# lis-epfl/apg_trajectory_tracking

Measured on AMD Instinct MI355X. Metric: env-steps/sec (fwd+bwd through dynamics), quad horizon=10 batch=65536, higher is better.
Workload: dtype f32; 1 GPU; quadrotor concurrent rollout fwd+bwd (dynamics + quad_mpc_loss + adjoint), BASELINE configs[1]; batch_per_gpu=65536, global_batch=65536, horizon=10, layout=packed, buffer_sets=20, input_bytes_all_sets=587202560, grad_state0=False, loss_mode=deferred, launch=hip-graph replays of the K steps, <= 1000 steps per graph, replays=3, parallelism=batch-sharded x1, no data-path collective

## Files before the change

### apg_trajectory_tracking_amd/_capi.py

```python
import ctypes
import os

import torch

_HERE = os.path.dirname(os.path.abspath(__file__))
LIB_PATH = os.environ.get("APG_LIB") or os.path.join(_HERE, "csrc", "libapg_hip.so")

LAYOUT_SOA = 0
LAYOUT_AOS = 1
LAYOUT_PACKED = 2
MAX_HORIZON = 48
ROLLOUT_BLOCK = 64

_c_float_p = ctypes.c_void_p


class ApgQuadParams(ctypes.Structure):
    _fields_ = [
        ("mass", ctypes.c_float),
        ("kinv", ctypes.c_float * 3),
        ("inertia", ctypes.c_float * 3),
        ("gravity", ctypes.c_float * 3),
        ("trans_drag", ctypes.c_float * 3),
        ("rot_drag", ctypes.c_float * 3),
# ... 257 lines not shown
        _I, _P, _P],
    "apg_wing_learnt_step_bwd": [
        _P, _P, _F, ctypes.POINTER(ApgWingParams), ctypes.POINTER(ctypes.c_float),
        _I, _P, _P, _P, _P, _P, _P],
    "apg_wing_learnt_rollout_workspace_floats": [_I],
    "apg_wing_learnt_rollout_fwd_bwd": [
        _P, _P, _P, _F, ctypes.POINTER(ApgWingLearnt),
        ctypes.POINTER(ApgWingLossWeights), _I, _I, _I, _P, _P, _P, _P, _P, _P, _P],
    "apg_wing_learnt_fit_grad_count": [],
    "apg_wing_learnt_fit_workspace_floats": [_I],
    "apg_wing_learnt_fit_fwd_bwd": [
        _P, _P, _F, ctypes.POINTER(ApgWingLearnt), _P, ctypes.POINTER(ApgWingParams),
        _F, _I, _P, _P, _P, _P, _P],
    "apg_wing_mlp_closed_loop": [
        _P, _I, _P, _F, ctypes.POINTER(ApgWingParams), ctypes.POINTER(ctypes.c_float),
        ctypes.POINTER(ApgLearntResidual),
        ctypes.POINTER(ApgWingPolicy), ctypes.POINTER(ctypes.c_float),
        ctypes.POINTER(ctypes.c_float), _F, _I, _I, _I, _F, _F, _I, _P, _P, _P,
        _P, _P, _P, _P, _P],
    "apg_planes_gemm_workspace_floats": [_I, _I, _I, _I],
    "apg_planes_gemm_default_wgs": [_I, _I, _I, _I],
    "apg_planes_gemm_multi_workspace_floats": [ctypes.POINTER(ApgGemmProblem), _I],
    "apg_planes_gemm_multi": [ctypes.POINTER(ApgGemmProblem), _I, _P, _P],
    "apg_planes_gemm": [_P, _I, _I, _P, _P, _I, _I, _I, _I,
                        ctypes.c_longlong, _P, _I, _P, _I, _P, _P],
    "apg_wing_step_fwd": [_P, _P, _F, ctypes.POINTER(ApgWingParams), _I, _I,
                          _P, _P],
    "apg_wing_step_bwd": [_P, _P, _F, ctypes.POINTER(ApgWingParams), _I, _I,
                          _P, _P, _P, _P],
    "apg_wing_rollout_fwd_bwd": [
        _P, _P, _P, _F, ctypes.POINTER(ApgWingParams),
        ctypes.POINTER(ApgWingLossWeights), _I, _I, _I, _P, _P, _P, _P, _P,
        ctypes.POINTER(ApgDeferredLoss), _P],
    "apg_wing_rollout_fwd": [_P, _P, _F, ctypes.POINTER(ApgWingParams), _I,
                             _I, _I, _P, _P],
    "apg_wing_set_two_per_lane": [_I],
    "apg_cartpole_step_fwd": [_P, _P, _F, ctypes.POINTER(ApgCartpoleParams),
                              _I, _I, _P, _P],
    "apg_cartpole_step_bwd": [_P, _P, _F, ctypes.POINTER(ApgCartpoleParams),
                              _I, _I, _P, _P, _P, _P],
    "apg_cartpole_rollout_fwd_bwd": [
        _P, _P, _F, ctypes.POINTER(ApgCartpoleParams), _I, _I, _I, _P, _P,
        _P, _P, _P, _P],
    "apg_cartpole_rollout_fwd": [_P, _P, _F, ctypes.POINTER(ApgCartpoleParams),
                                 _I, _I, _I, _P, _P],
    "apg_cartpole_policy_workspace_floats": [],
    "apg_cartpole_mlp_closed_loop": [
        _P, _F, ctypes.POINTER(ApgCartpoleParams), ctypes.POINTER(ApgCartpolePolicy),
        _I, _I, _I, _F, _I, _P, _P, _P, _P, _P, _P, _P, _P],
    "apg_cartpole_learnt_param_count": [],
    "apg_cartpole_learnt_workspace_floats": [_I],
    "apg_cartpole_learnt_step_fwd": [_P, _P, _F, ctypes.POINTER(ApgCartpoleLearnt), _I,
                                     _P, _P],
    "apg_cartpole_learnt_step_bwd": [_P, _P, _F, ctypes.POINTER(ApgCartpoleLearnt), _I,
                                     _P, _P, _P, _P, _P, _P],
    "apg_cartpole_learnt_rollout_fwd_bwd": [
        _P, _P, _F, ctypes.POINTER(ApgCartpoleLearnt), _I, _I, _I, _P, _P, _P, _P, _P,
        _P],
    "apg_cartpole_learnt_mlp_closed_loop": [
        _P, _F, ctypes.POINTER(ApgCartpoleLearnt), ctypes.POINTER(ApgCartpolePolicy),
        _I, _I, _I, _F, _I, _P, _P, _P, _P, _P, _P, _P, _P],
    "apg_quad_mpc_solve": [
        _P, _P, _I, _F, ctypes.POINTER(ApgQuadParams),
        ctypes.POINTER(ApgQuadLossWeights), ctypes.POINTER(ApgQuadMpcOptions), _I, _I,
        _P, _P, _P, _P],
    "apg_quad_mpc_closed_loop": [
        ctypes.POINTER(ApgQuadFlight), _F, ctypes.POINTER(ApgQuadParams),
        ctypes.POINTER(ApgLearntResidual), ctypes.POINTER(ApgQuadParams),
        ctypes.POINTER(ApgQuadLossWeights), ctypes.POINTER(ApgQuadMpcOptions), _I, _I,
        _P, _P, _P],
    "apg_quad_mpc_workspace_floats": [],
    "apg_cartpole_mpc_solve": [
        _P, _P, _F, ctypes.POINTER(ApgCartpoleParams),
        ctypes.POINTER(ApgCartpoleMpcOptions), _I, _I, _P, _P, _P, _P],
    "apg_cartpole_mpc_closed_loop": [
        _P, _F, ctypes.POINTER(ApgCartpoleParams), ctypes.POINTER(ApgCartpoleLearnt),
        ctypes.POINTER(ApgCartpoleParams), ctypes.POINTER(ApgCartpoleMpcOptions),
        _I, _I, _I, _I, _F, _I, _P, _P, _P, _P, _P, _P, _P, _P],
    "apg_reduce_loss_partials": [_P, _I, _P, _P],
    "apg_loss_partials_count": [_I],
    "apg_stream_copy": [_P, _P, ctypes.c_longlong, _P],
    "apg_stream_copy_shape": [_P, _P, ctypes.c_longlong, _I, _P],
    "apg_stream_rows_probe": [_P, ctypes.c_longlong, _P, ctypes.c_longlong, _I, _P],
    "apg_version": [],
    "apg_last_error_string": [],
}
_RESTYPES = {"apg_last_error_string": ctypes.c_char_p,
             "apg_planes_gemm_multi_workspace_floats": ctypes.c_longlong,
             "apg_quad_mlp_step_partials_floats": ctypes.c_longlong,
             "apg_quad_mlp_rollout_step_partials_floats": ctypes.c_longlong,
             "apg_linear_wgrad_workspace_floats": ctypes.c_longlong}

_lib = None


def lib():
    global _lib
    if _lib is None:
        if not os.path.exists(LIB_PATH):
            raise RuntimeError(
                f"{LIB_PATH} not found: build it with "
                "`python -m apg_trajectory_tracking_amd.build` "
                "(there is no CPU / PyTorch fallback for the APG kernels)")
        handle = ctypes.CDLL(LIB_PATH)
        for name, argtypes in SIGNATURES.items():
            fn = getattr(handle, name)
            fn.argtypes = argtypes
            fn.restype = _RESTYPES.get(name, ctypes.c_int)
        _lib = handle
    return _lib


def check(code, what):
    if code != 0:
        msg = lib().apg_last_error_string().decode()
        exc = ValueError if code == -1 else RuntimeError
        raise exc(f"{what} failed ({code}): {msg}")


def ptr(t):
    return None if t is None else t.data_ptr()


def stream_of(t):
    return torch.cuda.current_stream(t.device).cuda_stream


def require_device(*tensors):
    dev = None
    for t in tensors:
        if t is None:
            continue
        if not t.is_cuda:
            raise RuntimeError(
                "apg_trajectory_tracking_amd kernels run on an MI355X only: "
                f"got a tensor on {t.device} (no CPU fallback exists)")
        if t.dtype != torch.float32:
            raise TypeError(f"fp32 tensors required, got {t.dtype}")
        if not t.is_contiguous():
            raise ValueError("contiguous tensors required")
        if dev is None:
            dev = t.device
        elif t.device != dev:
            raise RuntimeError("all tensors must live on the same device")
    return dev


def loss_partials_count(B):
    return 1 if B <= 0 else (B + ROLLOUT_BLOCK - 1) // ROLLOUT_BLOCK
```

### apg_trajectory_tracking_amd/csrc/apg_device.h

```cpp
#pragma once
#include <hip/hip_runtime.h>
#include <stdint.h>

#include "apg.h"

#if !defined(APG_EXPERIMENT_BUILD) &&                                          \
    (defined(APG_STAMP) || defined(APG_QX) || defined(APG_EXP_NO_STORES) ||    \
     defined(APG_TRIG_1WORD) || defined(APG_SW_TRIG) || defined(APG_MLP_EXP) || \
     defined(APG_ROWS_BLOCK) || defined(APG_ROWS_ACT_PRE) ||                   \
     defined(APG_ROWS_REF_PER_STEP) || defined(APG_ROWS_REF_LOOK) ||           \
     defined(APG_ROWS_ST_AUX) || defined(APG_ROWS_REF_TOP) ||                  \
     defined(APG_ROWS_LD_AUX) || defined(APG_ROWS_STORE_AT_END) || defined(APG_ROWS_STORE_FLUSH_AT) ||                                               \
     defined(APG_REG_ACT_PRE) || defined(APG_REG_REF_PER_STEP) ||              \
     defined(APG_REG_REF_LOOK) || defined(APG_GEMM_ST_MAX) ||                  \
     defined(APG_GEMM_STREAM) || defined(APG_WING_WAVES) ||                    \
     defined(APG_WING_GROUP_PREFETCH) || defined(APG_WING_LITERALS) ||        \
     defined(APG_WING_PK) || defined(APG_WING_PK_KMODE))
#error "experiment macro in a product build (variants: -DAPG_EXPERIMENT_BUILD, tools/build_variant.py)"
#endif

namespace apg {

constexpr int kWave = 64;

// ... 122 lines not shown
  const float kf = rintf(x * 0.6366197466850281f);
  const int k = (int)kf;
  float r = fmaf(-kf, 1.5707963705062866f, x);
  r = fmaf(-kf, -4.371138828673793e-08f, r);
  r = fmaf(-kf, -1.7151245100058819e-15f, r);
  const float t = r * r;
  float ps = fmaf(t, 2.6658919978217455e-06f, -0.0001983463589567691f);
  ps = fmaf(t, ps, 0.008333319798111916f);
  ps = fmaf(t, ps, -0.1666666716337204f);
  const float s = fmaf(r * t, ps, r);
  float pc = fmaf(t, -4.336599204179947e-07f, 2.494495674909558e-05f);
  pc = fmaf(t, pc, -0.0013889188412576914f);
  pc = fmaf(t, pc, 0.0416666679084301f);
  const float c = fmaf(t * t, pc, fmaf(t, -0.5f, 1.0f));
  const bool swap = (k & 1) != 0;
  const float so = swap ? c : s, co = swap ? s : c;
  *sn = __builtin_bit_cast(
      float, __builtin_bit_cast(unsigned, so) ^ ((unsigned)(k & 2) << 30));
  *cs = __builtin_bit_cast(
      float, __builtin_bit_cast(unsigned, co) ^ ((unsigned)((k + 1) & 2) << 30));
}

__host__ __device__ __forceinline__ void sincos_hw(float x, float *sn, float *cs) {
#if defined(__HIP_DEVICE_COMPILE__)
  const float kHi = 0.15915494f;
  const float u = x * kHi;
#if defined(APG_TRIG_1WORD)
  const float f = __builtin_amdgcn_fractf(u);
#else
  const float kLo = 6.4206382e-09f;
  float e = fmaf(x, kHi, -u);
  e = fmaf(x, kLo, e);
  const float f = __builtin_amdgcn_fractf(u) + e;
#endif
  *sn = __builtin_amdgcn_sinf(f);
  *cs = __builtin_amdgcn_cosf(f);
#else
  *sn = (float)sin((double)x);
  *cs = (float)cos((double)x);
#endif
}

__host__ __device__ __forceinline__ float rcp_nr(float x) {
#if defined(__HIP_DEVICE_COMPILE__)
  const float r = __builtin_amdgcn_rcpf(x);
#else
  const float r = 1.0f / x;
#endif
  return fmaf(fmaf(-x, r, 1.0f), r, r);
}

__host__ __device__ __forceinline__ float rcp_nr_finite(float x) {
  const float kMax = 3.402823466e+38f;
#if defined(__HIP_DEVICE_COMPILE__)
  float r = __builtin_amdgcn_fmed3f(__builtin_amdgcn_rcpf(x), -kMax, kMax);
  r = fmaf(fmaf(-x, r, 1.0f), r, r);
  return __builtin_amdgcn_fmed3f(r, -kMax, kMax);
#else
  float r = fminf(fmaxf(1.0f / x, -kMax), kMax);
  r = fmaf(fmaf(-x, r, 1.0f), r, r);
  return fminf(fmaxf(r, -kMax), kMax);
#endif
}

__host__ __device__ __forceinline__ float sqrt_fast(float x) {
#if defined(__HIP_DEVICE_COMPILE__)
  return __builtin_amdgcn_sqrtf(x);
#else
  return sqrtf(x);
#endif
}

typedef float fx2 __attribute__((ext_vector_type(2)));
__host__ __device__ __forceinline__ fx2 rcp_nr(fx2 x) {
  return (fx2){rcp_nr(x.x), rcp_nr(x.y)};
}
__host__ __device__ __forceinline__ fx2 rcp_nr_finite(fx2 x) {
  return (fx2){rcp_nr_finite(x.x), rcp_nr_finite(x.y)};
}
__host__ __device__ __forceinline__ fx2 sqrt_fast(fx2 x) {
  return (fx2){sqrt_fast(x.x), sqrt_fast(x.y)};
}

__device__ __forceinline__ float wave_sum(float v) {
#pragma unroll
  for (int off = 32; off > 0; off >>= 1) v += __shfl_xor(v, off, kWave);
  return v;
}

__device__ __forceinline__ void write_wave_partial(float *partials, float lane_loss,
                                                   int count = 0x7fffffff) {
  float s = wave_sum(lane_loss);
  if ((threadIdx.x & (kWave - 1)) == 0) {
    int wave = (blockIdx.x * blockDim.x + threadIdx.x) / kWave;
    if (wave < count) partials[wave] = s;
  }
}

struct PrevPartials {
  float v[16];
  double acc;
};

__device__ __forceinline__ void reduce_prev_head(const ApgDeferredLoss &d,
                                                 PrevPartials &pp) {
  const int lane = threadIdx.x & (kWave - 1);
  pp.acc = 0.0;
  for (int base = 16 * kWave; base < d.prev_count; base += 16 * kWave) {
    float t[16];
#pragma unroll
    for (int j = 0; j < 16; ++j) {
      const int i = base + j * kWave + lane;
      t[j] = i < d.prev_count ? d.prev_partials[i] : 0.f;
    }
#pragma unroll
    for (int j = 0; j < 16; ++j) pp.acc += (double)t[j];
  }
#pragma unroll
  for (int j = 0; j < 16; ++j) {
    const int i = j * kWave + lane;
    pp.v[j] = i < d.prev_count ? d.prev_partials[i] : 0.f;
  }
}

__device__ __forceinline__ void reduce_prev_tail(const ApgDeferredLoss &d,
                                                 const PrevPartials &pp) {
  double acc = pp.acc;
#pragma unroll
  for (int j = 0; j < 16; ++j) acc += (double)pp.v[j];
#pragma unroll
  for (int off = 32; off > 0; off >>= 1) acc += __shfl_xor(acc, off, kWave);
  if ((threadIdx.x & (kWave - 1)) == 0) d.prev_loss[0] = (float)acc;
}

__device__ __forceinline__ void reduce_prev_partials(const ApgDeferredLoss &d) {
  PrevPartials pp;
  reduce_prev_head(d, pp);
  reduce_prev_tail(d, pp);
}

int launch_reduce_partials(const float *partials, int n, float *loss,
                           hipStream_t stream);

}
```

### apg_trajectory_tracking_amd/csrc/cartpole.hip

```cpp
#include "apg_device.h"
#include "cartpole_math.h"

namespace apg {
namespace {

template <int LAYOUT>
__global__ __launch_bounds__(256) void cart_step_fwd_kernel(
    const float *__restrict__ state, const float *__restrict__ action,
    CartConst c, int B, float *__restrict__ next) {
  const int b = blockIdx.x * blockDim.x + threadIdx.x;
  if (b >= B) return;
  float s[4];
  load_state<LAYOUT, 4>(state, B, b, s);
  cart_step(s, action[b], c);
  store_state<LAYOUT, 4>(next, B, b, s);
}

template <int LAYOUT>
__global__ __launch_bounds__(256) void cart_step_bwd_kernel(
    const float *__restrict__ state, const float *__restrict__ action,
    CartConst c, int B, const float *__restrict__ grad_next,
    float *__restrict__ grad_state, float *__restrict__ grad_action) {
  const int b = blockIdx.x * blockDim.x + threadIdx.x;
  if (b >= B) return;
  float s[4], lam[4];
  load_state<LAYOUT, 4>(state, B, b, s);
  load_state<LAYOUT, 4>(grad_next, B, b, lam);
  const float xd = s[1], thd = s[3];
  CartAux x = cart_step(s, action[b], c);
  const float ga = cart_step_adjoint(lam, xd, thd, x, c);
  if (grad_state) store_state<LAYOUT, 4>(grad_state, B, b, lam);
  if (grad_action) grad_action[b] = ga;
}

struct CartRolloutArgs {
  const float *state0, *actions;
  float *loss_partials, *grad_actions, *grad_state0, *states_out;
  CartConst c;
  int B, H;
};

template <int LAYOUT>
__global__ __launch_bounds__(APG_ROLLOUT_BLOCK) void cart_rollout_kernel(
    CartRolloutArgs A) {
  extern __shared__ float stash[];
  const int lane = threadIdx.x;
  const int b = blockIdx.x * blockDim.x + threadIdx.x;
  const bool live = b < A.B;
  const int bb = live ? b : A.B - 1;
  const CartConst c = A.c;
  const int H = A.H;
  const float wq[4] = {0.f, 3.f, 10.f, 1.f};
  const double inv = H > 1 ? 1.0 / (double)(H - 1) : 0.0;
  auto ST = [&](int k, int i) -> float & {
    return stash[(k * 4 + i) * APG_ROLLOUT_BLOCK + lane];
  };
  float s0[4], s[4];
  load_state<LAYOUT, 4>(A.state0, A.B, bb, s0);
#pragma unroll
  for (int i = 0; i < 4; ++i) s[i] = s0[i];
  float loss = 0.f;
  for (int k = 0; k < H; ++k) {
    float a[1];
    load_seq<LAYOUT, 1>(A.actions, A.B, H, 1, bb, k, 0, a);
#pragma unroll
    for (int i = 0; i < 4; ++i) ST(k, i) = s[i];
    cart_step(s, a[0], c);
    if (A.states_out && live)
      store_seq<LAYOUT, 4>(A.states_out, A.B, H, 4, b, k, 0, s);
    const float f = k < H - 1 ? (float)(1.0 - inv * (double)k) : 0.f;
#pragma unroll
    for (int i = 0; i < 4; ++i) {
      float d = s[i] - s0[i] * f;
      loss += (d * d) * wq[i];
    }
    loss += 0.01f * a[0] * a[0];
  }
  write_wave_partial(A.loss_partials, live ? loss : 0.f, (A.B + kWave - 1) / kWave);

  float lam[4] = {0.f, 0.f, 0.f, 0.f}, g0[4] = {0.f, 0.f, 0.f, 0.f};
  float nxt[4] = {s[0], s[1], s[2], s[3]};
  for (int k = H - 1; k >= 0; --k) {
    float a[1], pre[4];
    load_seq<LAYOUT, 1>(A.actions, A.B, H, 1, bb, k, 0, a);
    const float f = k < H - 1 ? (float)(1.0 - inv * (double)k) : 0.f;
#pragma unroll
    for (int i = 0; i < 4; ++i) {
      pre[i] = ST(k, i);
      float seed = 2.f * wq[i] * (nxt[i] - s0[i] * f);
      lam[i] += seed;
      g0[i] -= seed * f;
    }
    float tmp[4] = {pre[0], pre[1], pre[2], pre[3]};
    CartAux x = cart_step(tmp, a[0], c);
    float ga[1] = {cart_step_adjoint(lam, pre[1], pre[3], x, c) +
                   0.02f * a[0]};
    if (live) store_seq<LAYOUT, 1>(A.grad_actions, A.B, H, 1, b, k, 0, ga);
#pragma unroll
    for (int i = 0; i < 4; ++i) nxt[i] = pre[i];
  }
  if (A.grad_state0 && live) {
#pragma unroll
    for (int i = 0; i < 4; ++i) lam[i] += g0[i];
    store_state<LAYOUT, 4>(A.grad_state0, A.B, b, lam);
  }
}

template <int LAYOUT>
__global__ __launch_bounds__(256) void cart_rollout_fwd_kernel(
    const float *__restrict__ state0, const float *__restrict__ actions,
    CartConst c, int B, int H, float *__restrict__ states_out) {
  const int b = blockIdx.x * blockDim.x + threadIdx.x;
  if (b >= B) return;
  float s[4];
  load_state<LAYOUT, 4>(state0, B, b, s);
  for (int k = 0; k < H; ++k) {
    float a[1];
    load_seq<LAYOUT, 1>(actions, B, H, 1, b, k, 0, a);
    cart_step(s, a[0], c);
    store_seq<LAYOUT, 4>(states_out, B, H, 4, b, k, 0, s);
  }
}

inline int grid_for(int B, int block) { return (B + block - 1) / block; }

int check_args(const void *p0, const void *p1, const void *params, int B,
               int layout) {
  if (B < 0) { set_error("B must be >= 0 (got %d)", B); return APG_ERR_ARG; }
  if (layout != APG_LAYOUT_SOA && layout != APG_LAYOUT_AOS) {
    set_error("unknown layout %d", layout);
    return APG_ERR_ARG;
  }
  if (!params) { set_error("params is NULL"); return APG_ERR_ARG; }
  if (B > 0 && (!p0 || !p1)) { set_error("NULL input pointer"); return APG_ERR_ARG; }
  return APG_OK;
}

}
}

using namespace apg;

extern "C" {

int apg_cartpole_step_fwd(const float *state, const float *action, float dt,
                          const ApgCartpoleParams *params, int B, int layout,
                          float *next_state, apg_stream_t stream) {
  if (int e = check_args(state, action, params, B, layout)) return e;
  if (B == 0) return APG_OK;
  if (!next_state) { set_error("next_state is NULL"); return APG_ERR_ARG; }
  CartConst c = make_const(*params, dt);
  hipStream_t st = (hipStream_t)stream;
  if (layout == APG_LAYOUT_SOA)
    hipLaunchKernelGGL(cart_step_fwd_kernel<APG_LAYOUT_SOA>, dim3(grid_for(B, 256)),
                       dim3(256), 0, st, state, action, c, B, next_state);
  else
    hipLaunchKernelGGL(cart_step_fwd_kernel<APG_LAYOUT_AOS>, dim3(grid_for(B, 256)),
                       dim3(256), 0, st, state, action, c, B, next_state);
  return check_launch("cartpole_step_fwd");
}

// ... 81 lines not shown
```

### apg_trajectory_tracking_amd/csrc/cartpole_learnt.hip

```cpp
#include <stddef.h>

#include "apg_device.h"
#include "cartpole_learnt_math.h"

namespace apg {
namespace {

inline int grid_for(int B, int block) { return (B + block - 1) / block; }

constexpr int kStepBlock = 256;
constexpr int kStepWaves = kStepBlock / kWave;

__device__ __forceinline__ void stage_residual(float *rows, const ApgCartpoleLearnt &m) {
  for (int t = threadIdx.x; t < kCartResFloats; t += blockDim.x) {
    const int u = t / kCartResRow, j = t - u * kCartResRow;
    rows[t] = j < 5 ? m.w1[u * 5 + j] : j == 5 ? m.b1[u] : m.w2[(j - 6) * kCartResHidden + u];
  }
  __syncthreads();
}

__device__ __forceinline__ CartLearntParams load_params(const ApgCartpoleLearnt &m) {
  return CartLearntParams{*m.max_force_mag, *m.masspole, *m.length,
                          *m.friction,      *m.total_mass, *m.polemass_length};
}
// ... 50 lines not shown
    if (lane == 0) row[i] = v;
  }
  if (!res) {
    for (int i = kCartPhysGrads + lane; i < kCartLearntGrads; i += kWave) row[i] = 0.f;
    return;
  }
#pragma unroll
  for (int j = 0; j < 5; ++j) smp[wl][j][lane] = z[j];
#pragma unroll
  for (int o = 0; o < 4; ++o) smp[wl][5 + o][lane] = lam0[o];
  __syncthreads();
  float w[kCartResRow], gw[kCartResRow];
#pragma unroll
  for (int j = 0; j < kCartResRow; ++j) w[j] = rows[lane * kCartResRow + j], gw[j] = 0.f;
#pragma unroll 4
  for (int n = 0; n < kWave; ++n) {
    const float zn[5] = {smp[wl][0][n], smp[wl][1][n], smp[wl][2][n], smp[wl][3][n],
                         smp[wl][4][n]};
    const float ln[4] = {smp[wl][5][n], smp[wl][6][n], smp[wl][7][n], smp[wl][8][n]};
    cart_residual_unit_grads(w, zn, ln, gw);
  }
#pragma unroll
  for (int j = 0; j < 5; ++j) row[kCartGW1 + lane * 5 + j] = gw[j];
  row[kCartGB1 + lane] = gw[5];
#pragma unroll
  for (int o = 0; o < 4; ++o) row[kCartGW2 + o * kCartResHidden + lane] = gw[6 + o];
}

__global__ __launch_bounds__(256) void cart_learnt_reduce_kernel(
    const float *__restrict__ wave_partials, int waves, float *__restrict__ out) {
  const int i = blockIdx.x * blockDim.x + threadIdx.x;
  if (i >= kCartLearntGrads) return;
  float acc = 0.f;
  for (int w = 0; w < waves; ++w) acc += wave_partials[(size_t)w * kCartLearntGrads + i];
  out[i] = acc;
}

struct CartLearntRolloutArgs {
  const float *state0, *actions;
  float *loss_partials, *grad_actions, *grad_state0, *states_out;
  ApgCartpoleLearnt m;
  float dt;
  int B, H;
};

template <int LAYOUT>
__global__ __launch_bounds__(APG_ROLLOUT_BLOCK) void cart_learnt_rollout_kernel(
    CartLearntRolloutArgs A) {
  extern __shared__ float lds[];
  float *rows = lds, *stash = lds + kCartResFloats;
  stage_residual(rows, A.m);
  const int lane = threadIdx.x;
  const int b = blockIdx.x * blockDim.x + threadIdx.x;
  const bool live = b < A.B;
  const int bb = live ? b : A.B - 1;
  const CartConst c = make_learnt_const(load_params(A.m), A.dt);
  const int H = A.H;
  const float wq[4] = {0.f, 3.f, 10.f, 1.f};
  const double inv = H > 1 ? 1.0 / (double)(H - 1) : 0.0;
  auto ST = [&](int k, int i) -> float & {
    return stash[(k * 4 + i) * APG_ROLLOUT_BLOCK + lane];
  };
  float s0[4], s[4];
  load_state<LAYOUT, 4>(A.state0, A.B, bb, s0);
#pragma unroll
  for (int i = 0; i < 4; ++i) s[i] = s0[i];
  float loss = 0.f;
  for (int k = 0; k < H; ++k) {
    float a[1];
    load_seq<LAYOUT, 1>(A.actions, A.B, H, 1, bb, k, 0, a);
#pragma unroll
    for (int i = 0; i < 4; ++i) ST(k, i) = s[i];
    cart_learnt_step(s, a[0], c, rows);
    if (A.states_out && live)
      store_seq<LAYOUT, 4>(A.states_out, A.B, H, 4, b, k, 0, s);
    const float f = k < H - 1 ? (float)(1.0 - inv * (double)k) : 0.f;
#pragma unroll
    for (int i = 0; i < 4; ++i) {
      float d = s[i] - s0[i] * f;
      loss += (d * d) * wq[i];
    }
    loss += 0.01f * a[0] * a[0];
  }
  write_wave_partial(A.loss_partials, live ? loss : 0.f, (A.B + kWave - 1) / kWave);

  float lam[4] = {0.f, 0.f, 0.f, 0.f}, g0[4] = {0.f, 0.f, 0.f, 0.f};
  float nxt[4] = {s[0], s[1], s[2], s[3]};
  for (int k = H - 1; k >= 0; --k) {
    float a[1], pre[4];
    load_seq<LAYOUT, 1>(A.actions, A.B, H, 1, bb, k, 0, a);
    const float f = k < H - 1 ? (float)(1.0 - inv * (double)k) : 0.f;
#pragma unroll
    for (int i = 0; i < 4; ++i) {
      pre[i] = ST(k, i);
      float seed = 2.f * wq[i] * (nxt[i] - s0[i] * f);
      lam[i] += seed;
      g0[i] -= seed * f;
    }
    float tmp[4] = {pre[0], pre[1], pre[2], pre[3]};
    const CartAux x = cart_step(tmp, a[0], c);
    float ga[1] = {cart_learnt_step_adjoint(lam, pre, a[0], x, c, rows) + 0.02f * a[0]};
    if (live) store_seq<LAYOUT, 1>(A.grad_actions, A.B, H, 1, b, k, 0, ga);
#pragma unroll
    for (int i = 0; i < 4; ++i) nxt[i] = pre[i];
  }
  if (A.grad_state0 && live) {
#pragma unroll
    for (int i = 0; i < 4; ++i) lam[i] += g0[i];
    store_state<LAYOUT, 4>(A.grad_state0, A.B, b, lam);
  }
}

int check_model(const ApgCartpoleLearnt *m, bool need_residual) {
  if (!m) { set_error("model is NULL"); return APG_ERR_ARG; }
  if (!m->max_force_mag || !m->masspole || !m->length || !m->friction || !m->total_mass ||
      !m->polemass_length) {
    set_error("a physical parameter pointer is NULL");
    return APG_ERR_ARG;
  }
  const bool any = m->w1 || m->b1 || m->w2, all = m->w1 && m->b1 && m->w2;
  if (any != all || (need_residual && !all)) {
    set_error("w1 / b1 / w2 must be all given%s", need_residual ? "" : " or all NULL");
    return APG_ERR_ARG;
  }
  return APG_OK;
}

int check_step(const float *state, const float *action, const ApgCartpoleLearnt *m, int B) {
  if (B < 0) { set_error("B must be >= 0 (got %d)", B); return APG_ERR_ARG; }
  if (int e = check_model(m, false)) return e;
  if (B > 0 && (!state || !action)) { set_error("NULL input pointer"); return APG_ERR_ARG; }
  return APG_OK;
}

}
}

using namespace apg;

extern "C" {

int apg_cartpole_learnt_param_count(void) { return kCartLearntGrads; }

int apg_cartpole_learnt_workspace_floats(int B) {
  return B <= 0 ? 0 : grid_for(B, kStepBlock) * kStepWaves * kCartLearntGrads;
}

int apg_cartpole_learnt_step_fwd(const float *state, const float *action, float dt,
                                 const ApgCartpoleLearnt *model, int B, float *next_state,
                                 apg_stream_t stream) {
  if (int e = check_step(state, action, model, B)) return e;
  if (B == 0) return APG_OK;
  if (!next_state) { set_error("next_state is NULL"); return APG_ERR_ARG; }
  hipLaunchKernelGGL(cart_learnt_step_fwd_kernel, dim3(grid_for(B, kStepBlock)),
                     dim3(kStepBlock), 0, (hipStream_t)stream, state, action, *model, dt, B,
                     next_state);
  return check_launch("cartpole_learnt_step_fwd");
}

int apg_cartpole_learnt_step_bwd(const float *state, const float *action, float dt,
                                 const ApgCartpoleLearnt *model, int B,
                                 const float *grad_next, float *grad_state,
                                 float *grad_action, float *grad_params, float *workspace,
                                 apg_stream_t stream) {
  if (int e = check_step(state, action, model, B)) return e;
  if (!grad_params) { set_error("grad_params is NULL"); return APG_ERR_ARG; }
  hipStream_t st = (hipStream_t)stream;
// ... 67 lines not shown
```

### apg_trajectory_tracking_amd/csrc/common.hip

```cpp
#include <stdarg.h>
#include <stdio.h>

#include "apg_device.h"

namespace apg {

static thread_local char g_err[512] = "";

void set_error(const char *fmt, ...) {
  va_list ap;
  va_start(ap, fmt);
  vsnprintf(g_err, sizeof(g_err), fmt, ap);
  va_end(ap);
}

int device_slot() {
  int d = -1;
  return (hipGetDevice(&d) == hipSuccess && d >= 0 && d < kMaxDevices) ? d : -1;
}

int device_cu_count() {
  static int cus[kMaxDevices] = {};
  const int d = device_slot();
  if (d >= 0 && cus[d] > 0) return cus[d];
// ... 76 lines not shown
  }
  __syncthreads();
  const int x = threadIdx.x & 63, y = threadIdx.x >> 6;
  if (x < nb)
    for (int r = y; r < RC; r += 4) dst[(size_t)r * B + b0 + x] = tile[x * P + r];
}

}

typedef float f32x4_copy __attribute__((ext_vector_type(4)));
static __global__ __launch_bounds__(1024) void copy_flat_kernel(
    const f32x4_copy *__restrict__ src, f32x4_copy *__restrict__ dst, long long n16) {
  const long long i = (long long)blockIdx.x * blockDim.x + threadIdx.x;
  if (i < n16) dst[i] = src[i];
}
template <bool NT>
static __global__ __launch_bounds__(256) void copy_unroll4_kernel(
    const f32x4_copy *__restrict__ src, f32x4_copy *__restrict__ dst, long long n16) {
  const long long stride = (long long)gridDim.x * blockDim.x;
  long long i = (long long)blockIdx.x * blockDim.x + threadIdx.x;
  for (; i + 3 * stride < n16; i += 4 * stride) {
    const f32x4_copy a = src[i], b = src[i + stride], c = src[i + 2 * stride],
                     d = src[i + 3 * stride];
    if (NT) {
      __builtin_nontemporal_store(a, dst + i);
      __builtin_nontemporal_store(b, dst + i + stride);
      __builtin_nontemporal_store(c, dst + i + 2 * stride);
      __builtin_nontemporal_store(d, dst + i + 3 * stride);
    } else {
      dst[i] = a, dst[i + stride] = b, dst[i + 2 * stride] = c, dst[i + 3 * stride] = d;
    }
  }
  for (; i < n16; i += stride) dst[i] = src[i];
}

template <int SHAPE>
static __global__ __launch_bounds__(256) void stream_rows_probe_kernel(
    const f32x4_copy *__restrict__ in, f32x4_copy *__restrict__ out, long long in16,
    long long out16, int grp, int out_per_grp) {
  const long long i = (long long)blockIdx.x * blockDim.x + threadIdx.x;
  if (i >= in16) return;
  const f32x4_copy v = in[i];
  constexpr bool NT = SHAPE == 2 || SHAPE == 4;
  long long o;
  if (SHAPE <= 2) {
    o = i < out16 ? i : -1;
  } else {
    const long long g = i / grp;
    const int r = (int)(i - g * grp);
    o = r < out_per_grp ? g * out_per_grp + r : -1;
    if (o >= out16) o = -1;
  }
  if (o >= 0) {
    if (NT) __builtin_nontemporal_store(v, out + o);
    else out[o] = v;
  } else if (v.x + v.y == -1.2345e30f && v.z == 7.0f) {
    out[0] = v;
  }
}

static __global__ __launch_bounds__(64) void stream_rows_lane_kernel(const float *__restrict__ in,
                                                                    float *__restrict__ out,
                                                                    int B) {
  typedef unsigned u4_ __attribute__((ext_vector_type(4)));
  const int b = blockIdx.x * 64 + threadIdx.x;
  __amdgpu_buffer_rsrc_t ri =
      __builtin_amdgcn_make_buffer_rsrc((void *)in, 0, 28 * B * 16, 0x00020000);
  __amdgpu_buffer_rsrc_t ro = __builtin_amdgcn_make_buffer_rsrc((void *)out, 0, 10 * B * 16,
                                                                0x00020000);
  u4_ v[28];
#pragma unroll
  for (int i = 0; i < 28; ++i)
    v[i] = __builtin_amdgcn_raw_buffer_load_b128(ri, b * 16, i * B * 16, 0);
  u4_ acc = {0u, 0u, 0u, 0u};
#pragma unroll
  for (int i = 0; i < 28; ++i) acc += v[i];
#pragma unroll
  for (int i = 0; i < 10; ++i) {
    acc.x += i;
    __builtin_amdgcn_raw_buffer_store_b128(acc, ro, b * 16, i * B * 16, 2);
  }
}


extern "C" {

int apg_stream_rows_probe(const void *in, long long in_bytes, void *out, long long out_bytes,
                          int shape, apg_stream_t stream) {
  if (!in || !out || in_bytes <= 0 || out_bytes < 0 || (in_bytes & 15) || (out_bytes & 15) ||
      ((size_t)in & 15) || ((size_t)out & 15) || out_bytes > in_bytes) {
    apg::set_error("apg_stream_rows_probe: 16-byte aligned pointers and sizes, "
                   "0 <= out_bytes <= in_bytes expected");
    return APG_ERR_ARG;
  }
  if (shape < 1 || shape > 7) {
    apg::set_error("apg_stream_rows_probe: shape 1..7");
    return APG_ERR_ARG;
  }
  const long long in16 = in_bytes / 16, out16 = out_bytes / 16;
  if (shape == 7) {
    const long long B = in16 / 28;
    if (in16 % 28 || out16 != B * 10 || B % 64 || B > 0x3fffffll) {
      apg::set_error("apg_stream_rows_probe: shape 7 moves 28 input and 10 output rows of "
                     "B x 16 bytes, B a multiple of 64");
      return APG_ERR_ARG;
    }
    hipLaunchKernelGGL(stream_rows_lane_kernel, dim3((unsigned)(B / 64)), dim3(64), 0,
                       (hipStream_t)stream, (const float *)in, (float *)out, (int)B);
    return apg::check_launch("stream_rows_probe");
  }
  long long a = in16, b = out16 > 0 ? out16 : in16;
  while (b) { const long long t = a % b; a = b; b = t; }
  const long long grp = in16 / a, opg = out16 / a;
  if (grp > 0x7fffffffll) { apg::set_error("apg_stream_rows_probe: sizes"); return APG_ERR_ARG; }
  const int block = shape >= 5 ? 64 : 256;
  const long long blocks = (in16 + block - 1) / block;
  if (blocks > 0x7fffffffll) { apg::set_error("too large"); return APG_ERR_ARG; }
  hipStream_t st = (hipStream_t)stream;
  const f32x4_copy *s_ = (const f32x4_copy *)in;
  f32x4_copy *d_ = (f32x4_copy *)out;
#define APG_PROBE(S)                                                                        \
  hipLaunchKernelGGL(stream_rows_probe_kernel<S>, dim3((unsigned)blocks), dim3(block), 0, st, \
                     s_, d_, in16, out16, (int)grp, (int)opg)
  switch (shape) {
    case 1: case 5: APG_PROBE(1); break;
    case 2: case 6: APG_PROBE(2); break;
    case 3: APG_PROBE(3); break;
    default: APG_PROBE(4); break;
  }
#undef APG_PROBE
  return apg::check_launch("stream_rows_probe");
}

int apg_to_soa_multi(const ApgSoaItem *items, int n, int B, apg_stream_t stream) {
  if (!items || n < 1 || n > APG_SOA_MAX_ITEMS || B < 0) {
    apg::set_error("apg_to_soa_multi: need 1 <= n <= %d items, B >= 0",
                   APG_SOA_MAX_ITEMS);
    return APG_ERR_ARG;
  }
  apg::SoaArgs A;
  A.B = B;
  int max_r = 0;
  for (int i = 0; i < n; ++i) {
    const ApgSoaItem &q = items[i];
    if (q.R < 1 || q.ld < q.R) {
      apg::set_error("apg_to_soa: need B >= 0, R >= 1, ld >= R (item %d)", i);
      return APG_ERR_ARG;
    }
    if (B > 0 && (!q.src || !q.dst)) {
      apg::set_error("apg_to_soa: NULL pointer (item %d)", i);
      return APG_ERR_ARG;
    }
    A.it[i] = q;
    max_r = q.R > max_r ? q.R : max_r;
  }
  if (B == 0) return APG_OK;
  const int chunks = (max_r + apg::kSoaChunk - 1) / apg::kSoaChunk;
  if (chunks > 65535) {
    apg::set_error("apg_to_soa: R too large");
    return APG_ERR_ARG;
  }
  hipLaunchKernelGGL(apg::to_soa_kernel, dim3((B + 63) / 64, n, chunks), dim3(256), 0,
                     (hipStream_t)stream, A);
  return apg::check_launch("to_soa");
}

int apg_to_soa(const float *src, const long long *index, int B, int R, int ld,
               float *dst, apg_stream_t stream) {
// ... 86 lines not shown
```

### apg_trajectory_tracking_amd/csrc/lstm.hip

```cpp
#include "apg_device.h"
#include "policy_mfma.h"
#include "policy_mfma16.h"
#include "policy_tm.h"
#include "quad_math.h"
#include "learnt_residual.h"
#include "quad_flight.h"

namespace apg {
namespace {

constexpr int kH = 10;
constexpr int kRD = 9;
constexpr int kNF = 15;
constexpr int kNC = 20;
constexpr int kNP = kH - 2;
constexpr int kNX = kNF + kNC * kNP;
constexpr int kTau = kH + 3;
constexpr int kConvP = kNC * 2 * kTau;
constexpr int kConvPlanes = kConvP + kNC * kH;
constexpr int kNH = 8;
constexpr int kNG = 4 * kNH;
constexpr int kThreads = 256;
constexpr int kTrajPerBlock = kThreads / 2;

// ... 720 lines not shown
      run_g = fmaxf(run_g, amax);
      ex = scale_exponent(amax);
#pragma unroll
      for (int kb = 0; kb < 2; ++kb) {
        float v[8];
#pragma unroll
        for (int j = 0; j < 8; ++j) v[j] = __builtin_amdgcn_ldexpf(dG[8 * kb + j], -ex);
        xg[kb] = split8(v);
      }
    }
    f32x16 yh, yf;
#pragma unroll
    for (int i = 0; i < 16; ++i) yh[i] = 0.f, yf[i] = 0.f;
#pragma unroll
    for (int kb = 0; kb < 2; ++kb) {
      yh = mma3(L16.A(gA, mH + kb), xg[kb], yh);
      yf = mma3(L16.A(gA, mF + kb), xg[kb], yf);
    }
#pragma unroll
    for (int i = 0; i < 8; ++i) {
      yh[i] = __builtin_amdgcn_ldexpf(yh[i], ex);
      yf[i] = __builtin_amdgcn_ldexpf(yf[i], ex);
    }
#pragma unroll
    for (int r = 0; r < 4; ++r) dh[r] = yh[r];
    float dfeat[kNF], gs[12];
#pragma unroll
    for (int i = 0; i < 8; ++i) {
      const float own = yf[i], oth = other_half(own);
      dfeat[rrow(i)] = hi ? oth : own;
      if (rrow(i) + 4 < kNF) dfeat[rrow(i) + 4 < kNF ? rrow(i) + 4 : 0] = hi ? own : oth;
    }
    quad_features_adjoint(sc, t, dfeat, gs);
#pragma unroll
    for (int i = 0; i < 12; ++i) lam[i] += gs[i];
    float dpos[3] = {0.f, 0.f, 0.f};
#pragma unroll
    for (int eb = 0; eb < 5; ++eb) {
      f32x16 y0;
#pragma unroll
      for (int i = 0; i < 16; ++i) y0[i] = 0.f;
#pragma unroll
      for (int kb = 0; kb < 2; ++kb) y0 = mma3(L16.A(gA, mC + eb * 2 + kb), xg[kb], y0);
#pragma unroll
      for (int i = 0; i < 16; ++i) y0[i] = __builtin_amdgcn_ldexpf(y0[i], ex);
      const unsigned mws = hi ? mw[eb] >> 4 : mw[eb];
#pragma unroll
      for (int g = 0; g < 4; ++g) {
        const int ch = eb * 4 + g;
        float sum = 0.f;
#pragma unroll
        for (int ii = 0; ii < 4; ++ii) {
          const int i = 4 * g + ii;
          const float dcp = ((mws >> rrow(i)) & 1u) ? y0[i] : 0.f;
          dgn[ch][ii] += dcp;
          sum += dcp;
        }
        Pdc.st(vg, (unsigned)(ch * 2 * kTau + k + 3) * pB, dgn[ch][3]);
        dgn[ch][3] = dgn[ch][2], dgn[ch][2] = dgn[ch][1], dgn[ch][1] = dgn[ch][0];
        dgn[ch][0] = 0.f;
        Pdc.st(vb_lo, (unsigned)(kConvP + ch * kH + k) * pB, sum + other_half(sum));
#pragma unroll
        for (int q = 0; q < 3; ++q)
          dpos[q] = fmaf(L.U(gAq + (eb * 4 + g) * 3 + q), sum, dpos[q]);
      }
    }
#pragma unroll
    for (int q = 0; q < 3; ++q) lam[q] -= dpos[q] + other_half(dpos[q]);
  }
#pragma unroll
  for (int ch = 0; ch < kNC; ++ch)
#pragma unroll
    for (int tau = 0; tau < 3; ++tau)
      Pdc.st(vg, (unsigned)(ch * 2 * kTau + tau) * pitchB, dgn[ch][tau + 1]);
  if (st_lo && A.grad_state0)
#pragma unroll
    for (int i = 0; i < 12; ++i) A.grad_state0[(size_t)i * B + b] = lam[i];
  if (live && A.grad_h0)
#pragma unroll
    for (int r = 0; r < 4; ++r) A.grad_h0[(size_t)(r + 4 * hi) * B + b] = dh[r];
  if (live && A.grad_c0)
#pragma unroll
    for (int r = 0; r < 4; ++r) A.grad_c0[(size_t)(r + 4 * hi) * B + b] = dc[r];
  write_wave_partial(A.loss_partials, st_lo ? loss : 0.f);
  if (A.cot_amax) {
    float mg = run_g, mz = run_z;
#pragma unroll
    for (int s_ = 32; s_ >= 1; s_ >>= 1) {
      mg = fmaxf(mg, __shfl_xor(mg, s_, 64));
      mz = fmaxf(mz, __shfl_xor(mz, s_, 64));
    }
    const int group = blockIdx.x * (kThreads / 64) + wave;
    if (lane == 0 && group * 32 < B) A.cot_amax[2 * group] = mg, A.cot_amax[2 * group + 1] = mz;
  }
}

constexpr int kGwThreads = 512, kGwWaves = kGwThreads / 64, kGwGroups = 2;
constexpr int kGwBlocks = 5;
constexpr int kGwPart = kGwBlocks * 16 * 64;
constexpr int kGwTab = (hA + (nC + 2) * kBlock16) / 4;
constexpr int kGwActs = kNF + 3 * kNH;
#if !defined(APG_EXPERIMENT_BUILD) && defined(APG_GW_KNOCKOUT)
#error "experiment macro in a product build (variants: tools/build_policy_variant.sh)"
#endif
#ifndef APG_GW_KNOCKOUT
#define APG_GW_KNOCKOUT 0
#endif

struct GwArgs {
  const float *state0, *states, *in_ref;
  const float *acts;
  const float *d_gates, *d_zout;
  const float *cot_amax;
  const float *tables;
  float *partials;
  int B;
};

__device__ __forceinline__ void mask_tail(float (&v)[16], int hi, int nvalid) {
#pragma unroll
  for (int i = 0; i < 16; ++i)
    if (rrow(i) + 4 * hi >= nvalid) v[i] = 0.f;
}

__device__ __forceinline__ int amax_exponent(float m) {
  return m > 0.f && m < __builtin_inff() ? __builtin_amdgcn_frexp_expf(m) : 0;
}

struct GwLoads {
  TBlock tg, ta, tz;
  float pos[3];
};
constexpr int kGwSlots = 7;
constexpr int kGwWin = kGwSlots * 5 * kGwThreads;
constexpr int kGwBlk = kGwWaves * 2 * 1024;

template <int PH>
__device__ __forceinline__ void gate_wgrad_body(const GwArgs &A) {
  typedef __attribute__((address_space(3))) void *lds_ptr_t;
  extern __shared__ __attribute__((aligned(16))) float lds[];
  float *const win = lds + kGwTab;
  const int lane = threadIdx.x & 63, hi = lane >> 5, row = lane & 31;
  const int wave = __builtin_amdgcn_readfirstlane(threadIdx.x >> 6);
  const LdsView16 L16(lds, lane);
  float *const blk = lds + kGwTab + kGwWin + wave * 2048;
  const unsigned st_plane = (unsigned)lane >> 3, st_chunk = (((unsigned)lane & 7u) ^ st_plane) * 16u;
  auto staged = [&](int which, TBlock &t) {
#pragma unroll
    for (int g = 0; g < 4; ++g)
      t.q[g] = *reinterpret_cast<const u32x4 *>(
          blk + which * 1024 + (row * 8 + ((2 * g + hi) ^ (row & 7))) * 4);
  };
  const int B = A.B;
  const unsigned pitchB = (unsigned)B * 4u, pitchN = pitchB * kH;
  const Planes Ps0(A.state0, 12, pitchB), Pst(A.states, kH * 12, pitchB);
  const Planes Pin(A.in_ref, 2 * kH * kRD, pitchB);
  const Planes Pac(A.acts, kGwActs, pitchN), Pdg(A.d_gates, kNG, pitchN);
  const Planes Pdz(A.d_zout, 4, pitchN);
  const float cb = lds[hTbc + 2 * ((row & 3) + 4 * (row >> 3)) + ((row >> 2) & 1)];
  constexpr int kAuxCols = PH == 0 ? kNF + kNH : kNH, kAuxPlane0 = PH == 0 ? 0 : kNF + 2 * kNH;
  const bool aux_row = row < kAuxCols;
  const float a_one = row == kAuxCols ? 1.f : 0.f;

  f32x16 acc[kGwBlocks];
#pragma unroll
  for (int n = 0; n < kGwBlocks; ++n)
#pragma unroll
// ... 935 lines not shown
```

### apg_trajectory_tracking_amd/csrc/mlp_concurrent_fwd.h

```cpp
#pragma once
#include "mlp_common.h"

namespace apg {
namespace {


struct ConcArgs {
  const float *feat, *in_ref, *state0, *ref;
  float *x1, *h;
  unsigned *mask;
  float *d_zout;
  float *d_pre, *d_conv;
  float *states;
  float *loss_partials;
  const float *tables;
  float *xmax;
  QuadConst c;
  ApgQuadLossWeights w;
  int B, ref_cols, vel_col;
  const long long *index;
  long long n_rows;
  float *o_feat, *o_in_ref;
  int ld_feat, ld_in_ref, ld_state0, ld_ref;
  int win16;
// ... 259 lines not shown
#pragma unroll
    for (int i = 0; i < 12; ++i) s[i] = lds[zS0 + tl * kRowPadS + i];
  } else {
#pragma unroll
    for (int i = 0; i < 12; ++i) s[i] = Ps0.ld(vb, i * pN);
  }
  Trig st_trig[kH];
  float st_w[kH + 1][3], st_pv[kH][6];
#pragma unroll
  for (int k = 0; k < kH; ++k) {
#pragma unroll
    for (int i = 0; i < 3; ++i) st_w[k][i] = s[9 + i];
    st_trig[k] = make_trig(&s[3]);
    quad_step(s, act[k], c, st_trig[k]);
#pragma unroll
    for (int i = 0; i < 3; ++i) st_pv[k][i] = s[i], st_pv[k][3 + i] = s[6 + i];
#pragma unroll
    for (int i = 0; i < 12; ++i) Pst.st(vb_lo, (k * 12 + i) * pN, s[i]);
  }
#pragma unroll
  for (int i = 0; i < 3; ++i) st_w[kH][i] = s[9 + i];
  float loss = 0.f, lam[12];
#pragma unroll
  for (int i = 0; i < 12; ++i) lam[i] = 0.f;
  float rp[3], rv[3];
  const float *pr = lds + zRef + tl * kRowPadW;
  if (ROWS) {
    asm volatile("s_waitcnt vmcnt(0)" ::: "memory");
    __syncthreads();
  }
#pragma unroll
  for (int i = 0; i < 3; ++i) {
    rp[i] = ROWS ? pr[(kH - 1) * A.ref_cols + i]
                 : Prf.ld(vb, ((kH - 1) * A.ref_cols + i) * pN);
    rv[i] = ROWS ? pr[(kH - 1) * A.ref_cols + A.vel_col + i]
                 : Prf.ld(vb, ((kH - 1) * A.ref_cols + A.vel_col + i) * pN);
  }
#pragma unroll
  for (int k = kH - 1; k >= 0; --k) {
    float np_[3], nv_[3];
#pragma unroll
    for (int i = 0; i < 3; ++i) {
      np_[i] = k == 0 ? 0.f
               : ROWS ? pr[(k - 1) * A.ref_cols + i]
                      : Prf.ld(vb, ((k - 1) * A.ref_cols + i) * pN);
      nv_[i] = k == 0 ? 0.f
               : ROWS ? pr[(k - 1) * A.ref_cols + A.vel_col + i]
                      : Prf.ld(vb, ((k - 1) * A.ref_cols + A.vel_col + i) * pN);
    }
    float lp = 0.f, lv = 0.f, lw = 0.f, lr = 0.f;
#pragma unroll
    for (int i = 0; i < 3; ++i) {
      const float dp = st_pv[k][i] - rp[i], dv = st_pv[k][3 + i] - rv[i];
      const float wn = st_w[k + 1][i];
      lp += dp * dp, lv += dv * dv, lw += wn * wn;
      lam[i] += 2.f * A.w.pos * dp;
      lam[6 + i] += 2.f * A.w.vel * dv;
      lam[9 + i] += 2.f * A.w.av * wn;
    }
    const float a0 = act[k][0], da0 = a0 - 0.5f;
    float ga[4];
    ga[0] = 2.f * A.w.thrust * da0;
#pragma unroll
    for (int i = 1; i < 4; ++i) {
      const float d = act[k][i] - 0.5f;
      lr += d * d;
      ga[i] = 2.f * A.w.rates * d;
    }
    loss += A.w.pos * lp + A.w.vel * lv + A.w.av * lw + A.w.rates * lr +
            A.w.thrust * da0 * da0;
    quad_step_adjoint(lam, ga, a0, st_w[k], c, st_trig[k]);
#pragma unroll
    for (int i = 0; i < 4; ++i)
      act[k][i] = ga[i] * act[k][i] * (1.f - act[k][i]);
#pragma unroll
    for (int i = 0; i < 3; ++i) rp[i] = np_[i], rv[i] = nv_[i];
  }
#pragma unroll
  for (int cc = 0; cc < 20; ++cc) {
    const int row = khead(cc, 0);
    const float v = hi ? act[(row + 4) >> 2][(row + 4) & 3] : act[row >> 2][row & 3];
    Pdz.st(vr, row * pN, v);
  }
  write_wave_partial(A.loss_partials, st_lo ? loss : 0.f);
}

}
}
```

### apg_trajectory_tracking_amd/csrc/mlp_planes.hip

```cpp
#include "mlp_concurrent_fwd.h"
#include "apg_planes.h"

namespace apg {
namespace {
__global__ __launch_bounds__(256) void mlp_pack_cbwd_kernel(PackArgs A) {
  pack_cbwd(A, blockIdx.x * blockDim.x + threadIdx.x, gridDim.x * blockDim.x);
}

__global__ __launch_bounds__(256) void mlp_pack_pair_kernel(PackArgs A, int fwd_blocks) {
  if ((int)blockIdx.x < fwd_blocks) {
    pack_cfwd(A, blockIdx.x * blockDim.x + threadIdx.x, fwd_blocks * blockDim.x);
  } else {
    A.dst += kCfLds;
    pack_cbwd(A, (blockIdx.x - fwd_blocks) * blockDim.x + threadIdx.x,
              (gridDim.x - fwd_blocks) * blockDim.x);
  }
}

struct BwdArgs {
  const float *state0, *states, *actions, *ref, *x1, *h;
  const unsigned *mask;
  float *loss_partials;
  float *d_pre;
  float *d_zout;
// ... 110 lines not shown
    Op16 x[4];
    zero(e);
    int ex = scaled_split64(d, x);
    dense64T_16(e, x, L16, gA, m3T);
    __builtin_amdgcn_sched_barrier(0);
    tanh_adjoint(e, hv, Pdp, kW, vr, pN, ex);
    load_acts(hv, Ph, 0, vr, pN);
    __builtin_amdgcn_sched_barrier(0);
    zero(d);
    ex = scaled_split64(e, x);
    dense64T_16(d, x, L16, gA, m2T);
    __builtin_amdgcn_sched_barrier(0);
    tanh_adjoint(d, hv, Pdp, 0, vr, pN, ex);
    load_acts(hv, Px1, 0, vr, pN);
    __builtin_amdgcn_sched_barrier(0);
    zero(e);
    const int ex1 = scaled_split64(d, x);
    dense64T_16(e, x, L16, gA, m1sT);
    __builtin_amdgcn_sched_barrier(0);
    tanh_adjoint(e, hv, Pdp, 3 * kW, vr, pN, ex1);
    f32x16 f;
#pragma unroll
    for (int i = 0; i < 16; ++i) f[i] = 0.f;
    {
      Op16 xs[4];
      const int exs = scaled_split64(e, xs);
#pragma unroll
      for (int kb = 0; kb < 4; ++kb) f = mma3(L16.A(gA, mST + kb), xs[kb], f);
#pragma unroll
      for (int i = 0; i < 8; ++i) f[i] = __builtin_amdgcn_ldexpf(f[i], exs);
    }
    float dfeat[kNF], gs[12];
#pragma unroll
    for (int i = 0; i < 8; ++i) {
      const float own = f[i], oth = other_half(own);
      dfeat[rrow(i)] = hi ? oth : own;
      if (rrow(i) + 4 < kNF) dfeat[rrow(i) + 4 < kNF ? rrow(i) + 4 : 0] = hi ? own : oth;
    }
    quad_features_adjoint(sc, t, dfeat, gs);
#pragma unroll
    for (int i = 0; i < 12; ++i) lam[i] += gs[i];
    float dpos[3] = {0.f, 0.f, 0.f};
#pragma unroll
    for (int eb = 0; eb < 5; ++eb) {
      f32x16 y;
#pragma unroll
      for (int i = 0; i < 16; ++i) y[i] = 0.f;
#pragma unroll
      for (int kb = 0; kb < 4; ++kb) y = mma3(L16.A(gA, m1cT + eb * 4 + kb), x[kb], y);
#pragma unroll
      for (int i = 0; i < 16; ++i) y[i] = __builtin_amdgcn_ldexpf(y[i], ex1);
      const unsigned mws = hi ? mw[eb] >> 4 : mw[eb];
#pragma unroll
      for (int g = 0; g < 4; ++g) {
        const int ch = eb * 4 + g;
        float sum = 0.f;
#pragma unroll
        for (int ii = 0; ii < 4; ++ii) {
          const int i = 4 * g + ii;
          const float dcp = ((mws >> rrow(i)) & 1u) ? y[i] : 0.f;
          dgn[ch][ii] += dcp;
          sum += dcp;
        }
        Pdc.st(vg, (unsigned)(ch * 2 * kTau + k + 3) * pB, dgn[ch][3]);
        dgn[ch][3] = dgn[ch][2], dgn[ch][2] = dgn[ch][1], dgn[ch][1] = dgn[ch][0];
        dgn[ch][0] = 0.f;
        Pdc.st(vb_lo, (unsigned)(kConvP + ch * kH + k) * pB, sum + other_half(sum));
#pragma unroll
        for (int q = 0; q < 3; ++q)
          dpos[q] = fmaf(L.U(gAq + (eb * 4 + g) * 3 + q), sum, dpos[q]);
      }
    }
#pragma unroll
    for (int q = 0; q < 3; ++q) lam[q] -= dpos[q] + other_half(dpos[q]);
  }
#pragma unroll
  for (int ch = 0; ch < kNC; ++ch)
#pragma unroll
    for (int tau = 0; tau < 3; ++tau)
      Pdc.st(vg, (unsigned)(ch * 2 * kTau + tau) * pitchB, dgn[ch][tau + 1]);
  if (st_lo && A.grad_state0)
#pragma unroll
    for (int i = 0; i < 12; ++i) A.grad_state0[(size_t)i * B + b] = lam[i];
  write_wave_partial(A.loss_partials, st_lo ? loss : 0.f);
}

__global__ __launch_bounds__(kThreads) void mlp_concurrent_bwd_kernel(ConcArgs A) {
  extern __shared__ __attribute__((aligned(16))) float lds[];
  fill_lds(lds, A.tables, kCbLds);
  const int lane = threadIdx.x & 63, hi = lane >> 5;
  const LdsView L(lds, lane);
  const int wave = __builtin_amdgcn_readfirstlane(threadIdx.x >> 6);
  const int b = (blockIdx.x * (kThreads / 64) + wave) * 32 + (lane & 31);
  const int B = A.B;
  const bool live = b < B;
  const unsigned pN = (unsigned)B * 4u;
  const Planes Px1(A.x1, kN1, pN), Ph(A.h, 3 * kW, pN), Pmk(A.mask, 5, pN);
  const Planes Pdz(A.d_zout, kNA, pN), Pdp(A.d_pre, 4 * kW, pN);
  const Planes Pdc(A.d_conv, kNC * kNP, pN);
  const unsigned vb = live ? (unsigned)b * 4u : kDead;
  const unsigned vr = live ? vb + (hi ? 4u * pN : 0u) : kDead;

  float dzr[20];
#pragma unroll
  for (int cc = 0; cc < 20; ++cc) dzr[cc] = Pdz.ld(vr, khead(cc, 0) * pN);
  unsigned mw[5];
#pragma unroll
  for (int eb = 0; eb < 5; ++eb) mw[eb] = Pmk.ldu(vb, eb * pN);
  float hv[2][16];
  load_acts(hv, Ph, 2 * kW, vr, pN);
  __builtin_amdgcn_sched_barrier(0);
  const LdsView16 L16(lds, lane);
  f32x16 d[2], e[2];
  zero(d);
  int ex;
  {
    float amax = 0.f;
#pragma unroll
    for (int cc = 0; cc < 20; ++cc) amax = fmaxf(amax, fabsf(dzr[cc]));
    ex = scale_exponent(amax);
#pragma unroll
    for (int kb = 0; kb < 3; ++kb) {
      float v[8];
#pragma unroll
      for (int j = 0; j < 8; ++j)
        v[j] = kb * 8 + j < 20 ? __builtin_amdgcn_ldexpf(dzr[kb * 8 + j < 20 ? kb * 8 + j : 0], -ex)
                               : 0.f;
      const Op16 x = split8(v);
      d[0] = mma3(L16.A(gA, mOT + kb), x, d[0]);
      d[1] = mma3(L16.A(gA, mOT + 3 + kb), x, d[1]);
    }
  }
  __builtin_amdgcn_sched_barrier(0);
  tanh_adjoint(d, hv, Pdp, 2 * kW, vr, pN, ex);
  load_acts(hv, Ph, kW, vr, pN);
  __builtin_amdgcn_sched_barrier(0);
  Op16 x[4];
  zero(e);
  ex = scaled_split64(d, x);
  dense64T_16(e, x, L16, gA, m3T);
  __builtin_amdgcn_sched_barrier(0);
  tanh_adjoint(e, hv, Pdp, kW, vr, pN, ex);
  load_acts(hv, Ph, 0, vr, pN);
  __builtin_amdgcn_sched_barrier(0);
  zero(d);
  ex = scaled_split64(e, x);
  dense64T_16(d, x, L16, gA, m2T);
  __builtin_amdgcn_sched_barrier(0);
  tanh_adjoint(d, hv, Pdp, 0, vr, pN, ex);
  load_acts(hv, Px1, 0, vr, pN);
  __builtin_amdgcn_sched_barrier(0);
  zero(e);
  ex = scaled_split64(d, x);
  dense64T_16(e, x, L16, gA, m1sT);
  __builtin_amdgcn_sched_barrier(0);
  tanh_adjoint(e, hv, Pdp, 3 * kW, vr, pN, ex);
#pragma unroll
  for (int eb = 0; eb < 5; ++eb) {
    f32x16 y;
#pragma unroll
    for (int i = 0; i < 16; ++i) y[i] = 0.f;
#pragma unroll
    for (int kb = 0; kb < 4; ++kb) y = mma3(L16.A(gA, m1cT + eb * 4 + kb), x[kb], y);
    const unsigned mws = hi ? mw[eb] >> 4 : mw[eb];
#pragma unroll
    for (int i = 0; i < 16; ++i)
      Pdc.st(vr, (eb * 32 + rrow(i)) * pN,
// ... 128 lines not shown
```

### apg_trajectory_tracking_amd/csrc/mlp_rollout.hip

```cpp
#include "mlp_common.h"
#include "quad_flight.h"

namespace apg {
namespace {
template <bool XMAX, bool LEGACY = false>
__global__ __launch_bounds__(kThreads) void mlp_rollout_fwd_kernel(FwdArgs A) {
  extern __shared__ __attribute__((aligned(16))) float lds[];
  fill_lds(lds, A.tables, kCfLds);
  const LdsView16 L16(lds, threadIdx.x & 63);
  const int lane = threadIdx.x & 63, hi = lane >> 5;
  const LdsView L(lds, lane);
  const int wave = __builtin_amdgcn_readfirstlane(threadIdx.x >> 6);
  const int b = (blockIdx.x * (kThreads / 64) + wave) * 32 + (lane & 31);
  const int B = A.B;
  const bool live = b < B;
  const bool st_lo = live && hi == 0;
  const unsigned pitchB = (unsigned)B * 4u, pitchN = pitchB * kH;
  const QuadConst c = A.c;
  const Planes Ps0(A.state0, 12, pitchB), Pin(A.in_ref, 2 * kH * kRD, pitchB);
  const Planes Pst(A.states, kH * 12, pitchB), Pac(A.actions, kH * 4, pitchB);
  const Planes Pfe(A.feat, kNF, pitchN), Px1(A.x1, kN1, pitchN);
  const Planes Ph(A.h, 3 * kW, pitchN), Pmk(A.mask, 5, pitchN);
  const unsigned vb = live ? (unsigned)b * 4u : kDead;
  const unsigned vb_lo = st_lo ? vb : kDead;
// ... 824 lines not shown
        for (int i = 0; i < 16; ++i)
          v[i] = __builtin_amdgcn_fmed3f(v[i] - pv[i], -lim, lim);
        split16(v, fi - kPreXc, binr[jb]);
      }
    }
#pragma unroll 1
    for (int eb = 0; eb < 5; ++eb) {
      if (eb == 3) {
        ar_barrier();
        flush_add<6 * 1024>(lds, rg, part, (sFc1 + 4) * 4096, e1 + fc, bad);
        const int r_ = rg; rg = ro, ro = r_;
      }
      float xv[16];
      get_clamped(tx, xv, fc);
      if (eb < 4) tx.load(Px1, vtN, (unsigned)(kW + 32 * (eb + 1)) * pN + wcolN);
      int row_e = row, hi_e = hi;
      asm volatile("" : "+v"(row_e), "+v"(hi_e));
      {
        Op16 bx[2];
        split16(xv, fc - kPreX, bx);
        fc1_blocks(bx, lane_blk + rg + 2 * (eb < 3 ? eb : eb - 3) * 4096);
      }
      __builtin_amdgcn_sched_barrier(0);
      const char *tb = L16.b0 + gA + (a1c + 4 * eb) * kBlock16;
      f32x16 tt;
#pragma unroll
      for (int i = 0; i < 16; ++i) tt[i] = 0.f;
#pragma unroll
      for (int kb = 0; kb < 4; ++kb) {
        Op16 w;
        w.h = *reinterpret_cast<const u32x4 *>(tb + kb * kBlock16);
        w.l = *reinterpret_cast<const u32x4 *>(tb + kb * kBlock16 + 1024);
        tt = mma3(x1s[kb], w, tt);
      }
      int E1[16];
      texp(ex1, hi, E1);
      float v[16], sum = 0.f;
#pragma unroll
      for (int i = 0; i < 16; ++i) {
        v[i] = xv[i] > 0.f ? __builtin_amdgcn_ldexpf(tt[i], E1[i] - ec) : 0.f;
        sum += v[i];
      }
      char *cblk = lds + rConv + ((4 * (eb >> 1)) * 64 + 32 * (eb & 1)) * 4;
      sum += other_half(sum);
      sum += __builtin_bit_cast(float, __builtin_amdgcn_update_dpp(
          0, __builtin_bit_cast(int, sum), 0x111 , 0xf, 0xf, true)) *
             ((row_e & 7) >= 1 ? 1.f : 0.f);
      sum += __builtin_bit_cast(float, __builtin_amdgcn_update_dpp(
          0, __builtin_bit_cast(int, sum), 0x112 , 0xf, 0xf, true)) *
             ((row_e & 7) >= 2 ? 1.f : 0.f);
      sum += __builtin_bit_cast(float, __builtin_amdgcn_update_dpp(
          0, __builtin_bit_cast(int, sum), 0x114 , 0xf, 0xf, true)) *
             ((row_e & 7) >= 4 ? 1.f : 0.f);
      if (hi_e == 0 && (row_e & 7) == 7)
        gadd(part, (unsigned)(32 + 4 * eb + (row_e >> 3)) * 4u, bias_soff,
             bad ? __builtin_nanf("") : __builtin_amdgcn_ldexpf(sum, ec));
      Op16 ac[2];
      split16(v, -kPreDc, ac);
#pragma unroll
      for (int jb = 0; jb < 3; ++jb) {
        if (APG_AR_KNOCKOUT & 8) break;
        f32x16 acc;
#pragma unroll
        for (int i = 0; i < 16; ++i) acc[i] = 0.f;
#pragma unroll
        for (int kk = 0; kk < 2; ++kk) acc = mma3(ac[kk], binr[jb][kk], acc);
#pragma unroll
        for (int cc = 0; cc < 4; ++cc) {
          const int q = 32 * jb + row_e - kRD * (cc + 4 * hi_e);
          if (q >= 0 && q < 27) {
#pragma unroll
            for (int g = 0; g < 4; ++g) lds_add(cblk + (g * 64 + q) * 4, acc[4 * g + cc]);
          }
        }
      }
    }
    e5 = e1 + fc, ecv = ec + fi;
  }
  ar_barrier();
  flush_tail();
  if (st_lo && A.grad_state0)
#pragma unroll
    for (int i = 0; i < 12; ++i) A.grad_state0[(size_t)i * B + b] = lam[i];
  write_wave_partial(A.loss_partials, st_lo ? loss : 0.f);
}

}
}

using namespace apg;

extern "C" {

int apg_quad_mlp_workspace_floats(void) {
  return (kCfLds > kCbLds ? kCfLds : kCbLds) + kLearntFloats;
}

int apg_quad_mlp_loss_partials_count(int B) {
  return B <= 0 ? 0 : ((B + kTrajPerBlock - 1) / kTrajPerBlock) * (kThreads / kWave);
}

static int mlp_rollout_fwd(const float *state0, const float *in_ref, float dt,
                           const ApgQuadParams *params, const ApgMlpPolicy *policy, int B, int H,
                           float *states, float *actions, float *feat, float *x1, float *h,
                           unsigned *relu_mask, float *workspace, apg_stream_t stream,
                           bool legacy_inplace_ref);

int apg_quad_mlp_rollout_fwd(const float *state0, const float *in_ref, float dt,
                             const ApgQuadParams *params,
                             const ApgMlpPolicy *policy, int B, int H,
                             float *states, float *actions, float *feat,
                             float *x1, float *h, unsigned *relu_mask,
                             float *workspace, apg_stream_t stream) {
  return mlp_rollout_fwd(state0, in_ref, dt, params, policy, B, H, states, actions, feat, x1, h,
                         relu_mask, workspace, stream, false);
}

int apg_quad_mlp_rollout_fwd_inplace_ref(const float *state0, const float *in_ref, float dt,
                                         const ApgQuadParams *params,
                                         const ApgMlpPolicy *policy, int B, int H,
                                         float *states, float *actions, float *feat,
                                         float *x1, float *h, unsigned *relu_mask,
                                         float *workspace, apg_stream_t stream) {
  return mlp_rollout_fwd(state0, in_ref, dt, params, policy, B, H, states, actions, feat, x1, h,
                         relu_mask, workspace, stream, true);
}

static int mlp_rollout_fwd(const float *state0, const float *in_ref, float dt,
                           const ApgQuadParams *params, const ApgMlpPolicy *policy, int B, int H,
                           float *states, float *actions, float *feat, float *x1, float *h,
                           unsigned *relu_mask, float *workspace, apg_stream_t stream,
                           bool legacy_inplace_ref) {
  if (int e = check_mlp(params, policy, B, H)) return e;
  if (B == 0) return APG_OK;
  if (!state0 || !in_ref || !states || !actions || !feat || !x1 || !h ||
      !relu_mask || !workspace) {
    set_error("NULL buffer");
    return APG_ERR_ARG;
  }
  static PerDeviceOnce attr;
  if (!attr.test()) {
    if (int e = raise_lds(mlp_rollout_fwd_kernel<false>, kCfLds)) return e;
    if (int e = raise_lds(mlp_rollout_fwd_kernel<false, true>, kCfLds)) return e;
    attr.set();
  }
  FwdArgs A;
  A.state0 = state0, A.in_ref = in_ref, A.states = states, A.actions = actions;
  A.feat = feat, A.x1 = x1, A.h = h, A.mask = relu_mask;
  A.tables = workspace;
  A.xmax = nullptr;
  A.c = make_const(*params, dt);
  A.B = B;
  PackArgs P;
  P.pol = *policy, P.dst = workspace, P.head_rows = 4;
  hipLaunchKernelGGL(mlp_pack_cfwd_kernel, dim3((kCfLds + 255) / 256), dim3(256),
                     0, (hipStream_t)stream, P);
  const dim3 grid((B + kTrajPerBlock - 1) / kTrajPerBlock);
  if (legacy_inplace_ref)
    hipLaunchKernelGGL((mlp_rollout_fwd_kernel<false, true>), grid, dim3(kThreads),
                       kCfLds * sizeof(float), (hipStream_t)stream, A);
  else
    hipLaunchKernelGGL(mlp_rollout_fwd_kernel<false>, grid, dim3(kThreads),
                       kCfLds * sizeof(float), (hipStream_t)stream, A);
  return check_launch("quad_mlp_rollout_fwd");
}

int apg_quad_mlp_closed_loop(const ApgQuadFlight *flight, float dt, const ApgQuadParams *params,
// ... 152 lines not shown
```

### apg_trajectory_tracking_amd/csrc/quad.hip

```cpp
#include "apg_device.h"
#include "quad_math.h"

#ifndef APG_QX
#define APG_QX 0
#endif

namespace apg {
namespace {

#ifdef APG_STAMP
__device__ unsigned long long *g_stamps = nullptr;
#define APG_STAMP_DECL unsigned apg_stv = 0
#define APG_STAMP_PUT(i, t_)                                                   \
  asm volatile("v_writelane_b32 %0, %1, %3\nv_writelane_b32 %0, %2, %4"        \
               : "+v"(apg_stv)                                                 \
               : "s"((unsigned)(t_)), "s"((unsigned)((t_) >> 32)), "n"(2 * (i)), \
                 "n"(2 * (i) + 1))
#define APG_STAMP_AT(i)                                                        \
  do {                                                                         \
    __builtin_amdgcn_sched_barrier(0);                                         \
    unsigned long long t_;                                                     \
    asm volatile("s_memtime %0\ns_waitcnt lgkmcnt(0)" : "=s"(t_)::"memory");   \
    APG_STAMP_PUT(i, t_);                                                      \
    __builtin_amdgcn_sched_barrier(0);                                         \
  } while (0)
#define APG_STAMP_DEP(i, dep)                                                  \
  do {                                                                         \
    __builtin_amdgcn_sched_barrier(0);                                         \
    unsigned long long t_;                                                     \
    asm volatile("s_memtime %0\ns_waitcnt lgkmcnt(0)"                          \
                 : "=s"(t_)                                                    \
                 : "s"(dep)                                                    \
                 : "memory");                                                  \
    APG_STAMP_PUT(i, t_);                                                      \
    __builtin_amdgcn_sched_barrier(0);                                         \
  } while (0)
#define APG_STAMP_REAL(i)                                                      \
  do {                                                                         \
    __builtin_amdgcn_sched_barrier(0);                                         \
    unsigned long long t_;                                                     \
    asm volatile("s_memrealtime %0\ns_waitcnt lgkmcnt(0)" : "=s"(t_)::"memory"); \
    APG_STAMP_PUT(i, t_);                                                      \
    __builtin_amdgcn_sched_barrier(0);                                         \
  } while (0)
#define APG_STAMP_FLUSH()                                                      \
  do {                                                                         \
    asm volatile("s_waitcnt vmcnt(0)" ::: "memory");                           \
    APG_STAMP_AT(4);                                                           \
    APG_STAMP_REAL(5);                                                         \
    if (g_stamps && (threadIdx.x & 63) < 16)                                   \
      ((unsigned *)g_stamps)[(blockIdx.x * (blockDim.x / 64) + threadIdx.x / 64) * 16 + \
                             (threadIdx.x & 63)] = apg_stv;                    \
  } while (0)
#else
#define APG_STAMP_DECL
#define APG_STAMP_AT(i)
#define APG_STAMP_DEP(i, dep)
#define APG_STAMP_REAL(i)
#define APG_STAMP_FLUSH()
#endif

template <int LAYOUT>
__global__ __launch_bounds__(256) void quad_step_fwd_kernel(
    const float *__restrict__ state, const float *__restrict__ action,
    QuadConst c, int B, float *__restrict__ next) {
  const int b = blockIdx.x * blockDim.x + threadIdx.x;
  if (b >= B) return;
  float s[12], a[4];
  load_state<LAYOUT, 12>(state, B, b, s);
  load_state<LAYOUT, 4>(action, B, b, a);
  Trig t = make_trig(&s[3]);
  quad_step(s, a, c, t);
  store_state<LAYOUT, 12>(next, B, b, s);
}

template <int LAYOUT>
__global__ __launch_bounds__(256) void quad_step_bwd_kernel(
    const float *__restrict__ state, const float *__restrict__ action,
    QuadConst c, int B, const float *__restrict__ grad_next,
    float *__restrict__ grad_state, float *__restrict__ grad_action) {
  const int b = blockIdx.x * blockDim.x + threadIdx.x;
  if (b >= B) return;
  float s[12], a[4], lam[12];
  load_state<LAYOUT, 12>(state, B, b, s);
  load_state<LAYOUT, 4>(action, B, b, a);
  load_state<LAYOUT, 12>(grad_next, B, b, lam);
  Trig t = make_trig(&s[3]);
  float ga[4] = {0.f, 0.f, 0.f, 0.f};
  quad_step_adjoint(lam, ga, a[0], &s[9], c, t);
  if (grad_state) store_state<LAYOUT, 12>(grad_state, B, b, lam);
  if (grad_action) store_state<LAYOUT, 4>(grad_action, B, b, ga);
}

struct RolloutArgs {
  const float *state0, *actions, *ref;
  float *loss_partials, *grad_actions, *grad_state0, *states_out;
  QuadConst c;
  ApgQuadLossWeights w;
  ApgDeferredLoss prev;
  int B, H, ref_cols, vel_col;
};

template <int LAYOUT, int HT, bool STATES_OUT, bool BUF>
__global__ __launch_bounds__(APG_ROLLOUT_BLOCK) void quad_rollout_reg_kernel(
    RolloutArgs A) {
  static_assert(!BUF || LAYOUT == APG_LAYOUT_SOA, "buffer path is SoA only");
  APG_STAMP_DECL;
  APG_STAMP_AT(0);
  const int b = blockIdx.x * blockDim.x + threadIdx.x;
  const bool live = b < A.B;
  const int bb = live ? b : A.B - 1;
  const QuadConst c = A.c;
#ifndef APG_REG_ACT_PRE
#define APG_REG_ACT_PRE 3
#endif
#ifndef APG_REG_REF_PER_STEP
#define APG_REG_REF_PER_STEP 1
#endif
  constexpr int kActPre = HT < (APG_REG_ACT_PRE) ? HT : (APG_REG_ACT_PRE);
  constexpr int kRefPerStep = APG_REG_REF_PER_STEP;
#ifndef APG_REG_REF_LOOK
#define APG_REG_REF_LOOK 3
#endif
  constexpr int kRefLook = APG_REG_REF_LOOK > HT ? HT : APG_REG_REF_LOOK;

  const bool reducer = blockIdx.x == 0 && threadIdx.x < kWave &&
                       A.prev.prev_partials != nullptr;
  PrevPartials pp;
  if (reducer) reduce_prev_head(A.prev, pp);
  __builtin_amdgcn_sched_barrier(0);

  const SoaPlanes b_s0(A.state0, 12, A.B, bb), b_act(A.actions, HT * 4, A.B, bb),
      b_ref(A.ref, HT * A.ref_cols, A.B, bb),
      b_ga(A.grad_actions, HT * 4, A.B, bb),
      b_gs(A.grad_state0, 12, A.B, bb), b_so(A.states_out, HT * 12, A.B, bb);
  auto ld_ref = [&](int k, float(&p)[3], float(&v)[3]) {
    if constexpr (BUF) {
#pragma unroll
      for (int i = 0; i < 3; ++i) {
        p[i] = b_ref.ld(k * A.ref_cols + i);
        v[i] = b_ref.ld(k * A.ref_cols + A.vel_col + i);
      }
    } else {
      load_seq<LAYOUT, 3>(A.ref, A.B, HT, A.ref_cols, bb, k, 0, p);
      load_seq<LAYOUT, 3>(A.ref, A.B, HT, A.ref_cols, bb, k, A.vel_col, v);
    }
  };

  APG_STAMP_REAL(7);
  float s[12];
  float act[HT][4];
  float rp[HT][3], rv[HT][3];
  auto ld_act = [&](int k) {
    if constexpr (BUF) {
#pragma unroll
      for (int i = 0; i < 4; ++i) act[k][i] = b_act.ld(k * 4 + i);
    } else {
      load_seq<LAYOUT, 4>(A.actions, A.B, HT, 4, bb, k, 0, act[k]);
    }
  };
  if constexpr (BUF && (APG_QX & 4)) {
#pragma unroll
    for (int i = 3; i < 6; ++i) s[i] = b_s0.ld(i);
    __builtin_amdgcn_sched_barrier(0);
#pragma unroll
    for (int i = 9; i < 12; ++i) s[i] = b_s0.ld(i);
    __builtin_amdgcn_sched_barrier(0);
    ld_act(0);
    __builtin_amdgcn_sched_barrier(0);
#pragma unroll
    for (int i = 6; i < 9; ++i) s[i] = b_s0.ld(i);
#pragma unroll
    for (int i = 0; i < 3; ++i) s[i] = b_s0.ld(i);
    __builtin_amdgcn_sched_barrier(0);
#pragma unroll
    for (int k = 1; k < kActPre; ++k) {
      ld_act(k);
      __builtin_amdgcn_sched_barrier(0);
    }
  } else {
    if constexpr (BUF) {
#pragma unroll
      for (int i = 0; i < 12; ++i) s[i] = b_s0.ld(i);
    } else {
      load_state<LAYOUT, 12>(A.state0, A.B, bb, s);
    }
    __builtin_amdgcn_sched_barrier(0);
#pragma unroll
    for (int k = 0; k < kActPre; ++k) {
      ld_act(k);
      __builtin_amdgcn_sched_barrier(0);
    }
  }

  Trig st_trig[HT];
  float st_w[HT + 1][3];
  float st_pv[HT][6];
#pragma unroll
  for (int k = 0; k < HT; ++k) {
    {
      if (k + kActPre < HT) ld_act(k + kActPre);
      if constexpr (kRefLook == 0) {
#pragma unroll
        for (int j = 0; j < kRefPerStep; ++j) {
          const int kr = HT - 1 - (k * kRefPerStep + j);
          if (kr >= 0) ld_ref(kr, rp[kr], rv[kr]);
        }
      } else if (k >= HT - kRefLook) {
        const int kr = HT - 1 - (k - (HT - kRefLook));
        ld_ref(kr, rp[kr], rv[kr]);
      }
      __builtin_amdgcn_sched_barrier(0);
    }
#pragma unroll
    for (int i = 0; i < 3; ++i) st_w[k][i] = s[9 + i];
    st_trig[k] = make_trig(&s[3]);
    quad_step(s, act[k], c, st_trig[k]);
#pragma unroll
    for (int i = 0; i < 3; ++i) st_pv[k][i] = s[i], st_pv[k][3 + i] = s[6 + i];
    if constexpr (STATES_OUT) {
      if (live) {
        if constexpr (BUF) {
#pragma unroll
          for (int i = 0; i < 12; ++i) b_so.st(k * 12 + i, s[i]);
        } else {
          store_seq<LAYOUT, 12>(A.states_out, A.B, HT, 12, b, k, 0, s);
        }
      }
    }
    if (k == 0) APG_STAMP_AT(1);
  }
#pragma unroll
  for (int i = 0; i < 3; ++i) st_w[HT][i] = s[9 + i];
  APG_STAMP_AT(2);

  float sum_p = 0.f, sum_v = 0.f, sum_w = 0.f, sum_r = 0.f, sum_t = 0.f;
  const float wp2 = 2.f * A.w.pos, wv2 = 2.f * A.w.vel, ww2 = 2.f * A.w.av,
              wr2 = 2.f * A.w.rates, wt2 = 2.f * A.w.thrust;
  float lam[12];
#pragma unroll
  for (int i = 0; i < 12; ++i) lam[i] = 0.f;
#pragma unroll
  for (int k = HT - 1; k >= 0; --k) {
    if constexpr (kRefLook > 0) {
      if (k - kRefLook >= 0) ld_ref(k - kRefLook, rp[k - kRefLook], rv[k - kRefLook]);
      __builtin_amdgcn_sched_barrier(0);
    }
#pragma unroll
    for (int i = 0; i < 3; ++i) {
      const float dp = st_pv[k][i] - rp[k][i];
      const float dv = st_pv[k][3 + i] - rv[k][i];
      const float wn = st_w[k + 1][i];
      sum_p = fmaf(dp, dp, sum_p), sum_v = fmaf(dv, dv, sum_v);
      sum_w = fmaf(wn, wn, sum_w);
      lam[i] = fmaf(wp2, dp, lam[i]);
      lam[6 + i] = fmaf(wv2, dv, lam[6 + i]);
      lam[9 + i] = fmaf(ww2, wn, lam[9 + i]);
    }
    const float a0 = act[k][0], da0 = a0 - 0.5f;
    float ga[4];
    ga[0] = wt2 * da0;
    sum_t = fmaf(da0, da0, sum_t);
#pragma unroll
    for (int i = 1; i < 4; ++i) {
      const float d = act[k][i] - 0.5f;
      sum_r = fmaf(d, d, sum_r);
      ga[i] = wr2 * d;
    }
    quad_step_adjoint(lam, ga, a0, st_w[k], c, st_trig[k]);
    if (live) {
      if constexpr (BUF) {
#pragma unroll
        for (int i = 0; i < 4; ++i) b_ga.st(k * 4 + i, ga[i]);
      } else {
        store_seq<LAYOUT, 4>(A.grad_actions, A.B, HT, 4, b, k, 0, ga);
      }
    }
    if (k == HT / 2) APG_STAMP_AT(6);
  }
  if (A.grad_state0 && live) {
    if constexpr (BUF) {
#pragma unroll
      for (int i = 0; i < 12; ++i) b_gs.st(i, lam[i]);
    } else {
      store_state<LAYOUT, 12>(A.grad_state0, A.B, b, lam);
    }
  }
  APG_STAMP_AT(3);
  const float loss = A.w.pos * sum_p + A.w.vel * sum_v + A.w.av * sum_w +
                     A.w.rates * sum_r + A.w.thrust * sum_t;
  write_wave_partial(A.loss_partials, live ? loss : 0.f, (A.B + kWave - 1) / kWave);
  if (reducer) reduce_prev_tail(A.prev, pp);
  APG_STAMP_FLUSH();
}

struct RowArgs {
  float wd[3];
  ApgQuadLossWeights w;
  float *loss_partials, *grad_actions, *grad_state0, *states_out;
  ApgDeferredLoss prev;
};

typedef unsigned u4v __attribute__((ext_vector_type(4)));
typedef unsigned u2v __attribute__((ext_vector_type(2)));

__device__ __forceinline__ float u2f(unsigned u) { return __builtin_bit_cast(float, u); }
__device__ __forceinline__ unsigned f2u(float f) { return __builtin_bit_cast(unsigned, f); }

namespace rows_tune {
#ifdef APG_EXPERIMENT_BUILD
#define APG_ROWS_TUNE(frozen, knob) (knob)
#else
#define APG_ROWS_TUNE(frozen, knob) (frozen)
#endif
#ifndef APG_ROWS_BLOCK
#define APG_ROWS_BLOCK 64
#endif
#ifndef APG_ROWS_ACT_PRE
#define APG_ROWS_ACT_PRE 3
#endif
#ifndef APG_ROWS_REF_PER_STEP
#define APG_ROWS_REF_PER_STEP 1
#endif
#ifndef APG_ROWS_REF_LOOK
#define APG_ROWS_REF_LOOK 3
#endif
#ifndef APG_ROWS_ST_AUX
#define APG_ROWS_ST_AUX 2
#endif
#ifndef APG_ROWS_LD_AUX
#define APG_ROWS_LD_AUX 0
#endif
#ifndef APG_ROWS_STORE_AT_END
#define APG_ROWS_STORE_AT_END 1
#endif
#ifndef APG_ROWS_STORE_FLUSH_AT
#define APG_ROWS_STORE_FLUSH_AT (-1)
#endif
#ifndef APG_ROWS_REF_TOP
#define APG_ROWS_REF_TOP 0
#endif
constexpr int kBlock = APG_ROWS_TUNE(64, APG_ROWS_BLOCK);
constexpr int kActPreMax = APG_ROWS_TUNE(3, APG_ROWS_ACT_PRE);
constexpr int kRefPerStep = APG_ROWS_TUNE(1, APG_ROWS_REF_PER_STEP);
constexpr int kRefLookMax = APG_ROWS_TUNE(3, APG_ROWS_REF_LOOK);
constexpr int kStAux = APG_ROWS_TUNE(2, APG_ROWS_ST_AUX);
constexpr int kLdAux = APG_ROWS_TUNE(0, APG_ROWS_LD_AUX);
constexpr bool kStoreAtEnd = APG_ROWS_TUNE(1, APG_ROWS_STORE_AT_END) != 0;
constexpr int kStoreFlushAt = APG_ROWS_TUNE(-1, APG_ROWS_STORE_FLUSH_AT);
constexpr bool kRefTop = APG_ROWS_TUNE(0, APG_ROWS_REF_TOP) != 0;
#undef APG_ROWS_TUNE
}

template <int HT, bool STATES_OUT>
__global__ __launch_bounds__(rows_tune::kBlock) void quad_rollout_rows_kernel(
    const float *state0, const float *actions, const float *ref, int B, float dt,
    float half_dt, float half_dt2, float g0, float g1, float g2, float k0,
    float k1, float k2, RowArgs R) {
  APG_STAMP_DECL;
  APG_STAMP_AT(0);
  const int b = blockIdx.x * rows_tune::kBlock + threadIdx.x;
  const bool live = b < B;
  const int bb = live ? b : B - 1;
  using namespace rows_tune;
  constexpr int kActPre = HT < kActPreMax ? HT : kActPreMax;
  constexpr int kRefLook = kRefLookMax > HT ? HT : kRefLookMax;
  const auto r_s0 = __builtin_amdgcn_make_buffer_rsrc(
      const_cast<float *>(state0), 0, 3 * B * 16, 0x00020000);
  const auto r_act = __builtin_amdgcn_make_buffer_rsrc(
      const_cast<float *>(actions), 0, HT * B * 16, 0x00020000);
  const auto r_ref = __builtin_amdgcn_make_buffer_rsrc(
      const_cast<float *>(ref), 0, HT * B * 24, 0x00020000);
  const int v16 = bb * 16, v24 = bb * 24, p16 = B * 16, p24 = B * 24;
  APG_STAMP_REAL(7);

  u4v s4[3], a4[HT], rA[HT];
  u2v rB[HT];
  auto ld_ref = [&](int kr) {
    rA[kr] = __builtin_amdgcn_raw_buffer_load_b128(r_ref, v24, kr * p24, kLdAux);
    rB[kr] = __builtin_amdgcn_raw_buffer_load_b64(r_ref, v24 + 16, kr * p24, kLdAux);
  };
#pragma unroll
  for (int g = 0; g < 3; ++g)
    s4[g] = __builtin_amdgcn_raw_buffer_load_b128(r_s0, v16, g * p16, kLdAux);
  __builtin_amdgcn_sched_barrier(0);
#pragma unroll
  for (int k = 0; k < kActPre; ++k)
    a4[k] = __builtin_amdgcn_raw_buffer_load_b128(r_act, v16, k * p16, kLdAux);
  __builtin_amdgcn_sched_barrier(0);

  QuadConst c;
  c.dt = dt, c.half_dt = half_dt, c.half_dt2 = half_dt2;
  c.g[0] = g0, c.g[1] = g1, c.g[2] = g2;
  c.kdt[0] = k0, c.kdt[1] = k1, c.kdt[2] = k2;
  c.wd[0] = R.wd[0], c.wd[1] = R.wd[1], c.wd[2] = R.wd[2];
  const auto r_ga = __builtin_amdgcn_make_buffer_rsrc(R.grad_actions, 0,
                                                      HT * B * 16, 0x00020000);
  const int st16 = live ? b * 16 : (int)0x80000000;

  const bool reducer = blockIdx.x == 0 && threadIdx.x < kWave &&
                       R.prev.prev_partials != nullptr;
  PrevPartials pp;
  if (reducer) reduce_prev_head(R.prev, pp);
  __builtin_amdgcn_sched_barrier(0);

  float s[12];
  Trig st_trig[HT];
  float st_w[HT + 1][3];
  float st_pv[HT][6];
#pragma unroll
  for (int k = 0; k < HT; ++k) {
    {
      if (k + kActPre < HT)
        a4[k + kActPre] = __builtin_amdgcn_raw_buffer_load_b128(
            r_act, v16, (k + kActPre) * p16, kLdAux);
      if constexpr (kRefLook == 0) {
#pragma unroll
        for (int j = 0; j < kRefPerStep; ++j) {
          const int kr = HT - 1 - (k * kRefPerStep + j);
          if (kr >= 0) ld_ref(kr);
        }
      } else if (k >= HT - kRefLook) {
        ld_ref(HT - 1 - (k - (HT - kRefLook)));
      }
      __builtin_amdgcn_sched_barrier(0);
    }
    if (k == 0) {
#pragma unroll
      for (int g = 0; g < 3; ++g) {
        s[4 * g] = u2f(s4[g].x), s[4 * g + 1] = u2f(s4[g].y);
        s[4 * g + 2] = u2f(s4[g].z), s[4 * g + 3] = u2f(s4[g].w);
      }
    }
    const float act[4] = {u2f(a4[k].x), u2f(a4[k].y), u2f(a4[k].z), u2f(a4[k].w)};
#pragma unroll
    for (int i = 0; i < 3; ++i) st_w[k][i] = s[9 + i];
    st_trig[k] = make_trig(&s[3]);
    quad_step(s, act, c, st_trig[k]);
#pragma unroll
    for (int i = 0; i < 3; ++i) st_pv[k][i] = s[i], st_pv[k][3 + i] = s[6 + i];
    if constexpr (STATES_OUT) {
      const auto r_so = __builtin_amdgcn_make_buffer_rsrc(
          R.states_out, 0, HT * 3 * B * 16, 0x00020000);
#pragma unroll
      for (int g = 0; g < 3; ++g)
        __builtin_amdgcn_raw_buffer_store_b128(
            (u4v){f2u(s[4 * g]), f2u(s[4 * g + 1]), f2u(s[4 * g + 2]),
                  f2u(s[4 * g + 3])},
            r_so, st16, (k * 3 + g) * p16, 2);
    }
    if (k == 0) APG_STAMP_AT(1);
  }
#pragma unroll
  for (int i = 0; i < 3; ++i) st_w[HT][i] = s[9 + i];
  APG_STAMP_AT(2);

  float sum_p = 0.f, sum_v = 0.f, sum_w = 0.f, sum_r = 0.f, sum_t = 0.f;
  const float wp2 = 2.f * R.w.pos, wv2 = 2.f * R.w.vel, ww2 = 2.f * R.w.av,
              wr2 = 2.f * R.w.rates, wt2 = 2.f * R.w.thrust;
  float lam[12];
#pragma unroll
  for (int i = 0; i < 12; ++i) lam[i] = 0.f;
#pragma unroll
  for (int k = HT - 1; k >= 0; --k) {
    if constexpr (kRefLook > 0 && kRefTop) {
      if (k == HT - 1) {
#pragma unroll
        for (int kr = HT - 1 - kRefLook; kr >= 0; --kr) ld_ref(kr);
        __builtin_amdgcn_sched_barrier(0);
      }
    } else if constexpr (kRefLook > 0) {
      if (k - kRefLook >= 0) ld_ref(k - kRefLook);
      __builtin_amdgcn_sched_barrier(0);
    }
    const float rp[3] = {u2f(rA[k].x), u2f(rA[k].y), u2f(rA[k].z)};
    const float rv[3] = {u2f(rA[k].w), u2f(rB[k].x), u2f(rB[k].y)};
    const float act[4] = {u2f(a4[k].x), u2f(a4[k].y), u2f(a4[k].z), u2f(a4[k].w)};
#pragma unroll
    for (int i = 0; i < 3; ++i) {
      const float dp = st_pv[k][i] - rp[i];
      const float dv = st_pv[k][3 + i] - rv[i];
      const float wn = st_w[k + 1][i];
      sum_p = fmaf(dp, dp, sum_p), sum_v = fmaf(dv, dv, sum_v);
      sum_w = fmaf(wn, wn, sum_w);
      lam[i] = fmaf(wp2, dp, lam[i]);
      lam[6 + i] = fmaf(wv2, dv, lam[6 + i]);
      lam[9 + i] = fmaf(ww2, wn, lam[9 + i]);
    }
    const float a0 = act[0], da0 = a0 - 0.5f;
    float ga[4];
    ga[0] = wt2 * da0;
    sum_t = fmaf(da0, da0, sum_t);
#pragma unroll
    for (int i = 1; i < 4; ++i) {
      const float d = act[i] - 0.5f;
      sum_r = fmaf(d, d, sum_r);
      ga[i] = wr2 * d;
    }
    quad_step_adjoint(lam, ga, a0, st_w[k], c, st_trig[k]);
    if constexpr (kStoreAtEnd) {
      constexpr int kFlush = kStoreFlushAt;
      a4[k] = (u4v){f2u(ga[0]), f2u(ga[1]), f2u(ga[2]), f2u(ga[3])};
      if (k <= kFlush) {
        if (k == kFlush) {
#pragma unroll
          for (int j = HT - 1; j > kFlush; --j)
            __builtin_amdgcn_raw_buffer_store_b128(a4[j], r_ga, st16, j * p16, kStAux);
        }
        __builtin_amdgcn_raw_buffer_store_b128(a4[k], r_ga, st16, k * p16, kStAux);
      }
    } else {
      __builtin_amdgcn_raw_buffer_store_b128(
          (u4v){f2u(ga[0]), f2u(ga[1]), f2u(ga[2]), f2u(ga[3])}, r_ga, st16, k * p16,
          kStAux);
    }
    if (k == HT / 2) APG_STAMP_AT(6);
  }
  if constexpr (kStoreAtEnd && kStoreFlushAt < 0) {
#pragma unroll
    for (int k = HT - 1; k >= 0; --k)
      __builtin_amdgcn_raw_buffer_store_b128(a4[k], r_ga, st16, k * p16, kStAux);
  }
  if (R.grad_state0) {
    const auto r_gs = __builtin_amdgcn_make_buffer_rsrc(R.grad_state0, 0,
                                                        3 * B * 16, 0x00020000);
#pragma unroll
    for (int g = 0; g < 3; ++g)
      __builtin_amdgcn_raw_buffer_store_b128(
          (u4v){f2u(lam[4 * g]), f2u(lam[4 * g + 1]), f2u(lam[4 * g + 2]),
                f2u(lam[4 * g + 3])},
          r_gs, st16, g * p16, 2);
  }
  APG_STAMP_AT(3);
  const float loss = R.w.pos * sum_p + R.w.vel * sum_v + R.w.av * sum_w +
                     R.w.rates * sum_r + R.w.thrust * sum_t;
  write_wave_partial(R.loss_partials, live ? loss : 0.f, (B + kWave - 1) / kWave);
  if (reducer) reduce_prev_tail(R.prev, pp);
  APG_STAMP_FLUSH();
}

template <int HT, int RC, bool STATES_OUT>
__global__ __launch_bounds__(APG_ROLLOUT_BLOCK) void quad_rollout_aos_kernel(
    RolloutArgs A) {
  constexpr int kS0 = 64 * 12, kAct = 64 * 4 * HT;
  constexpr int kRefChunks = (64 * RC * HT * 4 + 1023) / 1024;
  constexpr int kVel = RC == 9 ? 6 : 3;
  __shared__ __attribute__((aligned(16))) float l_s0[kS0];
  __shared__ __attribute__((aligned(16))) float l_act[kAct];
  __shared__ __attribute__((aligned(16))) float l_ref[kRefChunks * 256];
  typedef __attribute__((address_space(3))) void *lds_ptr;
  const int lane = threadIdx.x;
  const int b = blockIdx.x * 64 + lane;
  const bool live = b < A.B;
  const QuadConst c = A.c;

  const bool reducer = blockIdx.x == 0 && threadIdx.x < kWave &&
                       A.prev.prev_partials != nullptr;
  PrevPartials pp;
  if (reducer) reduce_prev_head(A.prev, pp);

  const auto r_s0 = __builtin_amdgcn_make_buffer_rsrc(
      const_cast<float *>(A.state0), 0, A.B * 12 * 4, 0x00020000);
  const auto r_act = __builtin_amdgcn_make_buffer_rsrc(
      const_cast<float *>(A.actions), 0, A.B * HT * 4 * 4, 0x00020000);
  const auto r_ref = __builtin_amdgcn_make_buffer_rsrc(
      const_cast<float *>(A.ref), 0, A.B * HT * RC * 4, 0x00020000);
  const auto r_ga = __builtin_amdgcn_make_buffer_rsrc(
      A.grad_actions, 0, A.B * HT * 4 * 4, 0x00020000);
#pragma unroll
  for (int i = 0; i < 3; ++i)
    __builtin_amdgcn_raw_ptr_buffer_load_lds(
        r_s0, (lds_ptr)(l_s0 + i * 256), 16, lane * 16,
        blockIdx.x * (kS0 * 4) + i * 1024, 0, 0);
#pragma unroll
  for (int i = 0; i < HT; ++i)
    __builtin_amdgcn_raw_ptr_buffer_load_lds(
        r_act, (lds_ptr)(l_act + i * 256), 16, lane * 16,
        blockIdx.x * (kAct * 4) + i * 1024, 0, 0);
#pragma unroll
  for (int i = 0; i < kRefChunks; ++i)
    __builtin_amdgcn_raw_ptr_buffer_load_lds(
        r_ref, (lds_ptr)(l_ref + i * 256), 16, lane * 16,
        blockIdx.x * (64 * RC * HT * 4) + i * 1024, 0, 0);
  asm volatile("s_waitcnt vmcnt(%0)" ::"n"(kRefChunks) : "memory");

  float s[12];
#pragma unroll
  for (int i = 0; i < 3; ++i) {
    const float4 v = *reinterpret_cast<const float4 *>(&l_s0[lane * 12 + 4 * i]);
    s[4 * i] = v.x, s[4 * i + 1] = v.y, s[4 * i + 2] = v.z, s[4 * i + 3] = v.w;
  }
  Trig st_trig[HT];
  float st_w[HT + 1][3];
  float st_pv[HT][6];
#pragma unroll
  for (int k = 0; k < HT; ++k) {
    const float4 a4 =
        *reinterpret_cast<const float4 *>(&l_act[lane * 4 * HT + 4 * k]);
    const float a[4] = {a4.x, a4.y, a4.z, a4.w};
#pragma unroll
    for (int i = 0; i < 3; ++i) st_w[k][i] = s[9 + i];
    st_trig[k] = make_trig(&s[3]);
    quad_step(s, a, c, st_trig[k]);
#pragma unroll
    for (int i = 0; i < 3; ++i) st_pv[k][i] = s[i], st_pv[k][3 + i] = s[6 + i];
    if constexpr (STATES_OUT)
      if (live)
        store_seq<APG_LAYOUT_AOS, 12>(A.states_out, A.B, HT, 12, b, k, 0, s);
  }
#pragma unroll
  for (int i = 0; i < 3; ++i) st_w[HT][i] = s[9 + i];

  asm volatile("s_waitcnt vmcnt(0)" ::: "memory");

  float loss = 0.f;
  float lam[12];
#pragma unroll
  for (int i = 0; i < 12; ++i) lam[i] = 0.f;
#pragma unroll
  for (int k = HT - 1; k >= 0; --k) {
    const float *rrow = &l_ref[lane * RC * HT + k * RC];
    float4 a4 = *reinterpret_cast<const float4 *>(&l_act[lane * 4 * HT + 4 * k]);
    const float act[4] = {a4.x, a4.y, a4.z, a4.w};
    float lp = 0.f, lv = 0.f, lw = 0.f, lr = 0.f;
#pragma unroll
    for (int i = 0; i < 3; ++i) {
      const float dp = st_pv[k][i] - rrow[i];
      const float dv = st_pv[k][3 + i] - rrow[kVel + i];
      const float wn = st_w[k + 1][i];
      lp += dp * dp, lv += dv * dv, lw += wn * wn;
      lam[i] += 2.f * A.w.pos * dp;
      lam[6 + i] += 2.f * A.w.vel * dv;
      lam[9 + i] += 2.f * A.w.av * wn;
    }
    const float a0 = act[0], da0 = a0 - 0.5f;
    float ga[4];
    ga[0] = 2.f * A.w.thrust * da0;
#pragma unroll
    for (int i = 1; i < 4; ++i) {
      const float d = act[i] - 0.5f;
      lr += d * d;
      ga[i] = 2.f * A.w.rates * d;
    }
    loss += A.w.pos * lp + A.w.vel * lv + A.w.av * lw + A.w.rates * lr +
            A.w.thrust * da0 * da0;
    quad_step_adjoint(lam, ga, a0, st_w[k], c, st_trig[k]);
    *reinterpret_cast<float4 *>(&l_act[lane * 4 * HT + 4 * k]) =
        make_float4(ga[0], ga[1], ga[2], ga[3]);
  }
#pragma unroll
  for (int i = 0; i < HT; ++i) {
    const float4 v = *reinterpret_cast<const float4 *>(&l_act[i * 256 + lane * 4]);
    typedef float v4f __attribute__((ext_vector_type(4)));
    __builtin_amdgcn_raw_buffer_store_b128(
        __builtin_bit_cast(__attribute__((ext_vector_type(4))) unsigned,
                           (v4f){v.x, v.y, v.z, v.w}),
        r_ga, lane * 16, blockIdx.x * (kAct * 4) + i * 1024, 2);
  }
  if (A.grad_state0 && live)
    store_state<APG_LAYOUT_AOS, 12>(A.grad_state0, A.B, b, lam);
  write_wave_partial(A.loss_partials, live ? loss : 0.f, (A.B + kWave - 1) / kWave);
  if (reducer) reduce_prev_tail(A.prev, pp);
}

template <int LAYOUT, bool STATES_OUT>
__global__ __launch_bounds__(APG_ROLLOUT_BLOCK) void quad_rollout_lds_kernel(
    RolloutArgs A) {
  extern __shared__ float stash[];
  const int lane = threadIdx.x;
  const int b = blockIdx.x * blockDim.x + threadIdx.x;
  const bool live = b < A.B;
  const int bb = live ? b : A.B - 1;
  const QuadConst c = A.c;
  const int H = A.H;
  auto ST = [&](int k, int i) -> float & {
    return stash[(k * 12 + i) * APG_ROLLOUT_BLOCK + lane];
  };

  float s[12];
  load_state<LAYOUT, 12>(A.state0, A.B, bb, s);
  if (blockIdx.x == 0 && threadIdx.x < kWave && A.prev.prev_partials)
    reduce_prev_partials(A.prev);
  float loss = 0.f;
  for (int k = 0; k < H; ++k) {
    float a[4], rp[3], rv[3];
    load_seq<LAYOUT, 4>(A.actions, A.B, H, 4, bb, k, 0, a);
    load_seq<LAYOUT, 3>(A.ref, A.B, H, A.ref_cols, bb, k, 0, rp);
    load_seq<LAYOUT, 3>(A.ref, A.B, H, A.ref_cols, bb, k, A.vel_col, rv);
#pragma unroll
    for (int i = 0; i < 3; ++i) ST(k, i) = s[3 + i], ST(k, 3 + i) = s[9 + i];
    Trig t = make_trig(&s[3]);
    quad_step(s, a, c, t);
    if constexpr (STATES_OUT)
      if (live) store_seq<LAYOUT, 12>(A.states_out, A.B, H, 12, b, k, 0, s);
    float lp = 0.f, lv = 0.f, lw = 0.f;
#pragma unroll
    for (int i = 0; i < 3; ++i) {
      float dp = s[i] - rp[i], dv = s[6 + i] - rv[i];
      lp += dp * dp, lv += dv * dv, lw += s[9 + i] * s[9 + i];
      ST(k, 6 + i) = 2.f * A.w.pos * dp;
      ST(k, 9 + i) = 2.f * A.w.vel * dv;
    }
    float lr = 0.f;
#pragma unroll
    for (int i = 1; i < 4; ++i) lr += (a[i] - 0.5f) * (a[i] - 0.5f);
    const float da0 = a[0] - 0.5f;
    loss += A.w.pos * lp + A.w.vel * lv + A.w.av * lw + A.w.rates * lr +
            A.w.thrust * da0 * da0;
  }
  write_wave_partial(A.loss_partials, live ? loss : 0.f, (A.B + kWave - 1) / kWave);

  float lam[12], wn[3] = {s[9], s[10], s[11]};
#pragma unroll
  for (int i = 0; i < 12; ++i) lam[i] = 0.f;
  for (int k = H - 1; k >= 0; --k) {
    float a[4], att[3], w[3];
    load_seq<LAYOUT, 4>(A.actions, A.B, H, 4, bb, k, 0, a);
#pragma unroll
    for (int i = 0; i < 3; ++i) {
      att[i] = ST(k, i), w[i] = ST(k, 3 + i);
      lam[i] += ST(k, 6 + i);
      lam[6 + i] += ST(k, 9 + i);
      lam[9 + i] += 2.f * A.w.av * wn[i];
    }
    float ga[4] = {2.f * A.w.thrust * (a[0] - 0.5f),
                   2.f * A.w.rates * (a[1] - 0.5f),
                   2.f * A.w.rates * (a[2] - 0.5f),
                   2.f * A.w.rates * (a[3] - 0.5f)};
    Trig t = make_trig(att);
    quad_step_adjoint(lam, ga, a[0], w, c, t);
    if (live) store_seq<LAYOUT, 4>(A.grad_actions, A.B, H, 4, b, k, 0, ga);
#pragma unroll
    for (int i = 0; i < 3; ++i) wn[i] = w[i];
  }
  if (A.grad_state0 && live) store_state<LAYOUT, 12>(A.grad_state0, A.B, b, lam);
}

struct LearntArgs {
  const float *state0, *actions, *ref;
  float *loss_partials, *grad_actions, *grad_state0, *states_out;
  ApgLearntResidual m;
  QuadConst c;
  ApgQuadLossWeights w;
  int B, H, ref_cols, vel_col;
};

typedef __attribute__((address_space(4))) const float *cfloat_ptr;
struct LearntWeights {
  cfloat_ptr linear_at, w1, b1, w2, b2;
  __device__ explicit LearntWeights(const ApgLearntResidual &m)
      : linear_at((cfloat_ptr)m.linear_at), w1((cfloat_ptr)m.w1),
        b1((cfloat_ptr)m.b1), w2((cfloat_ptr)m.w2), b2((cfloat_ptr)m.b2) {}
};

#define APG_OPAQUE(p, v) asm volatile("" : "+s"(p), "+v"(v))
#define APG_OPAQUE16(p, v, o)                                                   \
  asm volatile(""                                                              \
               : "+s"(p), "+v"(v[o + 0]), "+v"(v[o + 1]), "+v"(v[o + 2]),      \
                 "+v"(v[o + 3]), "+v"(v[o + 4]), "+v"(v[o + 5]), "+v"(v[o + 6]), \
                 "+v"(v[o + 7]), "+v"(v[o + 8]), "+v"(v[o + 9]), "+v"(v[o + 10]), \
                 "+v"(v[o + 11]), "+v"(v[o + 12]), "+v"(v[o + 13]),            \
                 "+v"(v[o + 14]), "+v"(v[o + 15]))
__device__ __forceinline__ void learnt_hidden(const LearntWeights &m,
                                              const float (&x)[16], float (&z)[64]) {
  cfloat_ptr w1 = m.w1, b1 = m.b1;
  float x0 = x[0];
#pragma unroll
  for (int j = 0; j < 64; ++j) {
    if (j < 2) APG_OPAQUE(w1, x0);
    else APG_OPAQUE(w1, z[j - 2]);
    if (j % 16 == 0) APG_OPAQUE(b1, x0);
    float acc = b1[j];
#pragma unroll
    for (int i = 0; i < 16; ++i) acc = fmaf(w1[j * 16 + i], i == 0 ? x0 : x[i], acc);
    z[j] = acc;
  }
}

__device__ __forceinline__ void learnt_transform(const LearntWeights &m,
                                                 const float (&a)[4], float (&ap)[4]) {
  cfloat_ptr L = m.linear_at;
  float a0 = a[0];
  asm volatile("" : "+s"(L), "+v"(a0));
#pragma unroll
  for (int r = 0; r < 4; ++r)
    ap[r] = L[r * 4] * a0 + L[r * 4 + 1] * a[1] + L[r * 4 + 2] * a[2] +
            L[r * 4 + 3] * a[3];
}

__device__ __forceinline__ void learnt_step(float (&s)[12], const float (&a)[4],
                                            const LearntWeights &m,
                                            const QuadConst &c) {
  float ap[4], x[16], z[64], r[12];
// ... 36 lines not shown
  for (int i = 0; i < 12; ++i) x[i] = pre[i];
#pragma unroll
  for (int i = 0; i < 4; ++i) x[12 + i] = ap[i];
  learnt_hidden(m, x, z);
#pragma unroll
  for (int i = 0; i < 16; ++i) gx[i] = 0.f;
  cfloat_ptr w1 = m.w1, w2 = m.w2;
  float gh[64];
#pragma unroll
  for (int j = 0; j < 64; ++j) gh[j] = 0.f;
#pragma unroll
  for (int q = 0; q < 12; ++q) {
#pragma unroll
    for (int jb = 0; jb < 64; jb += 16) {
      APG_OPAQUE16(w2, gh, (jb + 32) % 64);
#pragma unroll
      for (int j = jb; j < jb + 16; ++j) gh[j] = fmaf(w2[q * 64 + j], lam[q], gh[j]);
    }
  }
  float gx2[32];
#pragma unroll
  for (int i = 0; i < 32; ++i) gx2[i] = 0.f;
#pragma unroll
  for (int j = 0; j < 64; ++j) {
    const int o = (j & 1) * 16;
    if (j & 1) APG_OPAQUE16(w1, gx2, 16);
    else APG_OPAQUE16(w1, gx2, 0);
    const float g = z[j] > 0.f ? gh[j] : 0.f;
#pragma unroll
    for (int i = 0; i < 16; ++i) gx2[o + i] = fmaf(w1[j * 16 + i], g, gx2[o + i]);
  }
#pragma unroll
  for (int i = 0; i < 16; ++i) gx[i] = gx2[i] + gx2[16 + i];
  const Trig t = make_trig(&pre[3]);
  float gap[4] = {0.f, 0.f, 0.f, 0.f};
  const float w[3] = {pre[9], pre[10], pre[11]};
  quad_step_adjoint(lam, gap, ap[0], w, c, t);
#pragma unroll
  for (int i = 0; i < 12; ++i) lam[i] += gx[i];
#pragma unroll
  for (int r = 0; r < 4; ++r) gap[r] += gx[12 + r];
  cfloat_ptr L = m.linear_at;
  asm volatile("" : "+s"(L), "+v"(gap[0]));
#pragma unroll
  for (int i = 0; i < 4; ++i)
    ga[i] += L[i] * gap[0] + L[4 + i] * gap[1] + L[8 + i] * gap[2] +
             L[12 + i] * gap[3];
}

template <int LAYOUT>
__global__ __launch_bounds__(64) void quad_learnt_rollout_kernel(LearntArgs A) {
  extern __shared__ float stash[];
  const int lane = threadIdx.x;
  const int b = blockIdx.x * 64 + lane;
  const bool live = b < A.B;
  const int bb = live ? b : A.B - 1;
  const QuadConst c = A.c;
  const int H = A.H;
  const LearntWeights W(A.m);
  auto ST = [&](int k, int i) -> float & { return stash[(k * 12 + i) * 64 + lane]; };
  float s[12];
  load_state<LAYOUT, 12>(A.state0, A.B, bb, s);
  float sum_p = 0.f, sum_v = 0.f, sum_w = 0.f, sum_r = 0.f, sum_t = 0.f;
  for (int k = 0; k < H; ++k) {
    float a[4], rp[3], rv[3];
    load_seq<LAYOUT, 4>(A.actions, A.B, H, 4, bb, k, 0, a);
    load_seq<LAYOUT, 3>(A.ref, A.B, H, A.ref_cols, bb, k, 0, rp);
    load_seq<LAYOUT, 3>(A.ref, A.B, H, A.ref_cols, bb, k, A.vel_col, rv);
#pragma unroll
    for (int i = 0; i < 12; ++i) ST(k, i) = s[i];
    learnt_step(s, a, W, c);
    if (A.states_out && live)
      store_seq<LAYOUT, 12>(A.states_out, A.B, H, 12, b, k, 0, s);
#pragma unroll
    for (int i = 0; i < 3; ++i) {
      const float dp = s[i] - rp[i], dv = s[6 + i] - rv[i], d = a[1 + i] - 0.5f;
      sum_p = fmaf(dp, dp, sum_p), sum_v = fmaf(dv, dv, sum_v);
      sum_w = fmaf(s[9 + i], s[9 + i], sum_w), sum_r = fmaf(d, d, sum_r);
    }
    sum_t = fmaf(a[0] - 0.5f, a[0] - 0.5f, sum_t);
  }
  const float loss = A.w.pos * sum_p + A.w.vel * sum_v + A.w.av * sum_w +
                     A.w.rates * sum_r + A.w.thrust * sum_t;
  write_wave_partial(A.loss_partials, live ? loss : 0.f, (A.B + kWave - 1) / kWave);

  float lam[12], nxt[12];
#pragma unroll
  for (int i = 0; i < 12; ++i) lam[i] = 0.f, nxt[i] = s[i];
  for (int k = H - 1; k >= 0; --k) {
    float a[4], rp[3], rv[3], pre[12];
    load_seq<LAYOUT, 4>(A.actions, A.B, H, 4, bb, k, 0, a);
    load_seq<LAYOUT, 3>(A.ref, A.B, H, A.ref_cols, bb, k, 0, rp);
    load_seq<LAYOUT, 3>(A.ref, A.B, H, A.ref_cols, bb, k, A.vel_col, rv);
#pragma unroll
    for (int i = 0; i < 3; ++i) {
      lam[i] += 2.f * A.w.pos * (nxt[i] - rp[i]);
      lam[6 + i] += 2.f * A.w.vel * (nxt[6 + i] - rv[i]);
      lam[9 + i] += 2.f * A.w.av * nxt[9 + i];
    }
#pragma unroll
    for (int i = 0; i < 12; ++i) pre[i] = ST(k, i);
    float ga[4] = {2.f * A.w.thrust * (a[0] - 0.5f), 2.f * A.w.rates * (a[1] - 0.5f),
                   2.f * A.w.rates * (a[2] - 0.5f), 2.f * A.w.rates * (a[3] - 0.5f)};
    learnt_step_adjoint(lam, ga, pre, a, W, c);
    if (live) store_seq<LAYOUT, 4>(A.grad_actions, A.B, H, 4, b, k, 0, ga);
#pragma unroll
    for (int i = 0; i < 12; ++i) nxt[i] = pre[i];
  }
  if (A.grad_state0 && live) store_state<LAYOUT, 12>(A.grad_state0, A.B, b, lam);
}

template <int LAYOUT>
__global__ __launch_bounds__(256) void quad_rollout_fwd_kernel(
    const float *__restrict__ state0, const float *__restrict__ actions,
    QuadConst c, int B, int H, float *__restrict__ states_out) {
  const int b = blockIdx.x * blockDim.x + threadIdx.x;
  if (b >= B) return;
  float s[12];
  load_state<LAYOUT, 12>(state0, B, b, s);
  for (int k = 0; k < H; ++k) {
    float a[4];
    load_seq<LAYOUT, 4>(actions, B, H, 4, b, k, 0, a);
    Trig t = make_trig(&s[3]);
    quad_step(s, a, c, t);
    store_seq<LAYOUT, 12>(states_out, B, H, 12, b, k, 0, s);
  }
}

template <int LAYOUT>
__global__ __launch_bounds__(APG_ROLLOUT_BLOCK) void quad_loss_kernel(
    const float *__restrict__ states, const float *__restrict__ ref,
    int ref_cols, int vel_col, const float *__restrict__ actions,
    ApgQuadLossWeights w, int B, int H, float *__restrict__ partials,
    float *__restrict__ grad_states, float *__restrict__ grad_actions) {
  const int b = blockIdx.x * blockDim.x + threadIdx.x;
  const bool live = b < B;
  const int bb = live ? b : B - 1;
  float loss = 0.f;
  for (int k = 0; k < H; ++k) {
    float s[12], a[4], rp[3], rv[3], gs[12], ga[4];
    load_seq<LAYOUT, 12>(states, B, H, 12, bb, k, 0, s);
    load_seq<LAYOUT, 4>(actions, B, H, 4, bb, k, 0, a);
    load_seq<LAYOUT, 3>(ref, B, H, ref_cols, bb, k, 0, rp);
    load_seq<LAYOUT, 3>(ref, B, H, ref_cols, bb, k, vel_col, rv);
    float lp = 0.f, lv = 0.f, lw = 0.f, lr = 0.f;
#pragma unroll
    for (int i = 0; i < 3; ++i) {
      float dp = s[i] - rp[i], dv = s[6 + i] - rv[i], d = a[1 + i] - 0.5f;
      lp += dp * dp, lv += dv * dv, lw += s[9 + i] * s[9 + i], lr += d * d;
      gs[i] = 2.f * w.pos * dp, gs[3 + i] = 0.f;
      gs[6 + i] = 2.f * w.vel * dv, gs[9 + i] = 2.f * w.av * s[9 + i];
      ga[1 + i] = 2.f * w.rates * d;
    }
    const float da0 = a[0] - 0.5f;
    ga[0] = 2.f * w.thrust * da0;
    loss += w.pos * lp + w.vel * lv + w.av * lw + w.rates * lr +
            w.thrust * da0 * da0;
    if (live && grad_states)
      store_seq<LAYOUT, 12>(grad_states, B, H, 12, b, k, 0, gs);
    if (live && grad_actions)
      store_seq<LAYOUT, 4>(grad_actions, B, H, 4, b, k, 0, ga);
  }
  write_wave_partial(partials, live ? loss : 0.f, (B + kWave - 1) / kWave);
}

template <int LAYOUT>
__global__ __launch_bounds__(256) void quad_features_fwd_kernel(
    const float *__restrict__ state, int B, float *__restrict__ feat) {
  const int b = blockIdx.x * blockDim.x + threadIdx.x;
  if (b >= B) return;
  float s[12], f[15];
  load_state<LAYOUT, 12>(state, B, b, s);
  quad_features(s, make_trig(&s[3]), f);
  store_state<LAYOUT, 15>(feat, B, b, f);
}

template <int LAYOUT>
__global__ __launch_bounds__(256) void quad_features_bwd_kernel(
    const float *__restrict__ state, const float *__restrict__ gfeat, int B,
    float *__restrict__ gstate) {
  const int b = blockIdx.x * blockDim.x + threadIdx.x;
  if (b >= B) return;
  float s[12], gf[15], gs[12];
  load_state<LAYOUT, 12>(state, B, b, s);
  load_state<LAYOUT, 15>(gfeat, B, b, gf);
  quad_features_adjoint(s, make_trig(&s[3]), gf, gs);
  store_state<LAYOUT, 12>(gstate, B, b, gs);
}

inline int grid_for(int B, int block) { return (B + block - 1) / block; }

int check_common(const void *p0, const void *p1, const void *params, int B,
                 int layout, bool packed_ok = false) {
  if (B < 0) { set_error("B must be >= 0 (got %d)", B); return APG_ERR_ARG; }
  if (layout != APG_LAYOUT_SOA && layout != APG_LAYOUT_AOS &&
      !(packed_ok && layout == APG_LAYOUT_PACKED)) {
    set_error("unknown layout %d", layout);
    return APG_ERR_ARG;
  }
  if (!params) { set_error("params is NULL"); return APG_ERR_ARG; }
  if (B > 0 && (!p0 || !p1)) { set_error("NULL input pointer"); return APG_ERR_ARG; }
  return APG_OK;
}

template <int LAYOUT, bool SO>
int launch_rollout(const RolloutArgs &A, hipStream_t st) {
  const dim3 grid(grid_for(A.B, APG_ROLLOUT_BLOCK)), block(APG_ROLLOUT_BLOCK);
  const bool buf_ok = (long long)A.H * 12 * A.B * 4 < (1ll << 31);
  if constexpr (LAYOUT == APG_LAYOUT_AOS) {
    if (buf_ok && (A.H == 5 || A.H == 10)) {
#define APG_AOS(HT, RC)                                                       \
  hipLaunchKernelGGL((quad_rollout_aos_kernel<HT, RC, SO>), grid, block, 0,  \
                     st, A)
      if (A.H == 10 && A.ref_cols == 9) APG_AOS(10, 9);
      else if (A.H == 10) APG_AOS(10, 6);
      else if (A.ref_cols == 9) APG_AOS(5, 9);
      else APG_AOS(5, 6);
#undef APG_AOS
      return check_launch("quad_rollout_fwd_bwd");
    }
  }
  switch (A.H) {
#define APG_CASE(HT)                                                          \
  case HT:                                                                    \
    if (LAYOUT == APG_LAYOUT_SOA && buf_ok)                                   \
      hipLaunchKernelGGL(                                                     \
          (quad_rollout_reg_kernel<LAYOUT, HT, SO, LAYOUT == APG_LAYOUT_SOA>), \
          grid, block, 0, st, A);                                             \
    else                                                                      \
      hipLaunchKernelGGL((quad_rollout_reg_kernel<LAYOUT, HT, SO, false>),    \
                         grid, block, 0, st, A);                              \
    break;
    APG_CASE(5) APG_CASE(10)
#undef APG_CASE
    default: {
      const size_t lds = (size_t)A.H * 12 * APG_ROLLOUT_BLOCK * sizeof(float);
      if (lds > 64 * 1024 &&
          hipFuncSetAttribute((const void *)quad_rollout_lds_kernel<LAYOUT, SO>,
                              hipFuncAttributeMaxDynamicSharedMemorySize,
                              (int)lds) != hipSuccess)
        return check_launch("hipFuncSetAttribute(quad_rollout_lds)");
      hipLaunchKernelGGL((quad_rollout_lds_kernel<LAYOUT, SO>), grid, block, lds,
                         st, A);
    }
  }
  return check_launch("quad_rollout_fwd_bwd");
// ... 297 lines not shown
```

### apg_trajectory_tracking_amd/csrc/wing.hip

```cpp
#include <stddef.h>
#include <stdlib.h>

#include "apg_device.h"
#include "wing_math.h"

namespace apg {
namespace {


template <int LAYOUT>
__global__ __launch_bounds__(256) void wing_step_fwd_kernel(
    const float *__restrict__ state, const float *__restrict__ action,
    WingConst k, int B, float *__restrict__ next) {
  const int b = blockIdx.x * blockDim.x + threadIdx.x;
  if (b >= B) return;
  float s[12], a[4];
  load_state<LAYOUT, 12>(state, B, b, s);
  load_state<LAYOUT, 4>(action, B, b, a);
  wing_step(s, a, k);
  store_state<LAYOUT, 12>(next, B, b, s);
}

template <int LAYOUT>
__global__ __launch_bounds__(256) void wing_step_bwd_kernel(
// ... 49 lines not shown
  if (!live) b_ga.voff = b_so.voff = b_gs.voff = (int)0x80000000;
  auto ld_act = [&](int kq, float(&o)[4]) {
    if constexpr (BUF) {
#pragma unroll
      for (int i = 0; i < 4; ++i) o[i] = b_act.ld(kq * 4 + i);
    } else {
      load_seq<LAYOUT, 4>(A.actions, A.B, A.H, 4, bb, kq, 0, o);
    }
  };
  auto ld_ref = [&](int kq, float(&o)[3]) {
    if constexpr (BUF) {
#pragma unroll
      for (int i = 0; i < 3; ++i) o[i] = b_ref.ld(kq * 3 + i);
    } else {
      load_seq<LAYOUT, 3>(A.ref, A.B, A.H, 3, bb, kq, 0, o);
    }
  };
  typedef __attribute__((address_space(4))) const WingConst *const_ptr;
  typedef __attribute__((address_space(4))) const char *const_bytes;
  const_ptr kp = (const_ptr)((const_bytes)__builtin_amdgcn_kernarg_segment_ptr() +
                             offsetof(WingRolloutArgs, k));
#define APG_LAUNDER(p) asm volatile("" : "+s"(p))
  const WingDefaultK kl;
  const float w_pos = LIT ? kWingDefaultPosWeight : A.w.pos,
              w_act = LIT ? kWingDefaultActionWeight : A.w.action;
  auto step = [&](float(&s_)[12], const float(&a_)[4]) {
    if constexpr (LIT) {
      wing_step(s_, a_, kl);
    } else {
      APG_LAUNDER(kp);
      wing_step(s_, a_, *kp);
    }
  };
  const int H = A.H, S = A.stride;
  auto ST = [&](int slot, int i) -> float & {
    return stash[(slot * 12 + i) * APG_ROLLOUT_BLOCK + lane];
  };
  float s[12];
  load_state<LAYOUT, 12>(A.state0, A.B, bb, s);
  if (blockIdx.x == 0 && threadIdx.x < kWave && A.prev.prev_partials)
    reduce_prev_partials(A.prev);
  float loss = 0.f;
  float a_q[2][4], r_q[2][3];
#pragma unroll
  for (int d = 0; d < 2; ++d) {
    const int kq = d < H ? d : H - 1;
    ld_act(kq, a_q[d]);
    ld_ref(kq, r_q[d]);
  }
  for (int kk = 0, slot = 0, phase = 0; kk < H; ++kk) {
    float a[4], rp[3];
#pragma unroll
    for (int i = 0; i < 4; ++i) a[i] = a_q[0][i], a_q[0][i] = a_q[1][i];
#pragma unroll
    for (int i = 0; i < 3; ++i) rp[i] = r_q[0][i], r_q[0][i] = r_q[1][i];
    {
      const int kq = kk + 2 < H ? kk + 2 : H - 1;
      ld_act(kq, a_q[1]);
      ld_ref(kq, r_q[1]);
    }
    if (phase == 0) {
#pragma unroll
      for (int i = 0; i < 12; ++i) ST(slot, i) = s[i];
      ++slot;
    }
    if (++phase == S) phase = 0;
    step(s, a);
    if (A.states_out) {
      if constexpr (BUF) {
#pragma unroll
        for (int i = 0; i < 12; ++i) b_so.st(kk * 12 + i, s[i]);
      } else if (live) {
        store_seq<LAYOUT, 12>(A.states_out, A.B, H, 12, b, kk, 0, s);
      }
    }
    float lp = 0.f, la = 0.f;
#pragma unroll
    for (int i = 0; i < 3; ++i) {
      float dp = s[i] - rp[i], d = a[1 + i] - 0.5f;
      lp += dp * dp, la += d * d;
    }
    loss += w_pos * lp + w_act * la;
  }
  write_wave_partial(A.loss_partials, live ? loss : 0.f, (A.B + kWave - 1) / kWave);

  float lam[12];
#pragma unroll
  for (int i = 0; i < 12; ++i) lam[i] = 0.f;
  float nxt[3] = {s[0], s[1], s[2]};
  const int G = (H + S - 1) / S;
  float act[kWingMaxStride][4], rpg[kWingMaxStride][3];
  float act_n[kWingMaxStride][4], rpg_n[kWingMaxStride][3];
  auto load_group = [&](int g, float(&ga_)[kWingMaxStride][4],
                        float(&gr_)[kWingMaxStride][3]) {
#pragma unroll
    for (int j = 0; j < kWingMaxStride; ++j) {
      int kq = g * S + j;
      kq = (j < S && kq < H) ? kq : H - 1;
      ld_act(kq, ga_[j]);
      ld_ref(kq, gr_[j]);
    }
  };
#if APG_WING_GROUP_PREFETCH
  load_group(G - 1, act, rpg);
#endif
  for (int g = G - 1; g >= 0; --g) {
    const int k0 = g * S;
    const int n = (H - k0) < S ? (H - k0) : S;
#if APG_WING_GROUP_PREFETCH
    load_group(g > 0 ? g - 1 : 0, act_n, rpg_n);
#else
    load_group(g, act, rpg);
#endif
    float pre[kWingMaxStride + 1][12];
#pragma unroll
    for (int i = 0; i < 12; ++i) pre[0][i] = ST(g, i);
#pragma unroll
    for (int j = 0; j < kWingMaxStride; ++j) {
      if (j < n) {
        if (j + 1 < kWingMaxStride && j + 1 < n) {
#pragma unroll
          for (int i = 0; i < 12; ++i) pre[j + 1][i] = pre[j][i];
          step(pre[j + 1], act[j]);
        }
      }
    }
#pragma unroll
    for (int j = kWingMaxStride - 1; j >= 0; --j) {
      if (j < n) {
        const int kk = k0 + j;
        float pn[3] = {nxt[0], nxt[1], nxt[2]}, sd[12];
        if (j + 1 < kWingMaxStride && j + 1 < n) {
#pragma unroll
          for (int i = 0; i < 3; ++i) pn[i] = pre[j + 1][i];
        }
#pragma unroll
        for (int i = 0; i < 3; ++i) lam[i] += 2.f * w_pos * (pn[i] - rpg[j][i]);
        float ga[4] = {0.f, 2.f * w_act * (act[j][1] - 0.5f),
                       2.f * w_act * (act[j][2] - 0.5f),
                       2.f * w_act * (act[j][3] - 0.5f)};
        WingAux x;
        if constexpr (LIT) {
          wing_rates(pre[j], act[j], kl, x, sd);
          wing_step_adjoint(lam, ga, pre[j], x, sd, kl);
        } else {
          APG_LAUNDER(kp);
          wing_rates(pre[j], act[j], *kp, x, sd);
          wing_step_adjoint(lam, ga, pre[j], x, sd, *kp);
        }
        if constexpr (BUF) {
#pragma unroll
          for (int i = 0; i < 4; ++i) b_ga.st(kk * 4 + i, ga[i]);
        } else if (live) {
          store_seq<LAYOUT, 4>(A.grad_actions, A.B, H, 4, b, kk, 0, ga);
        }
      }
    }
#pragma unroll
    for (int i = 0; i < 3; ++i) nxt[i] = pre[0][i];
#if APG_WING_GROUP_PREFETCH
#pragma unroll
    for (int j = 0; j < kWingMaxStride; ++j) {
#pragma unroll
      for (int i = 0; i < 4; ++i) act[j][i] = act_n[j][i];
#pragma unroll
      for (int i = 0; i < 3; ++i) rpg[j][i] = rpg_n[j][i];
    }
// ... 451 lines not shown
```

### apg_trajectory_tracking_amd/csrc/wing_learnt.hip

```cpp
#include <stddef.h>

#include "apg_device.h"
#include "wing_learnt_math.h"

namespace apg {
namespace {

inline int grid_for(int B, int block) { return (B + block - 1) / block; }

__global__ __launch_bounds__(256) void wing_learnt_step_fwd_kernel(
    const float *__restrict__ state, const float *__restrict__ action,
    WingGeneralConst k, int B, float *__restrict__ next) {
  const int b = blockIdx.x * blockDim.x + threadIdx.x;
  if (b >= B) return;
  float s[12], a[4];
  load_state<APG_LAYOUT_AOS, 12>(state, B, b, s);
  load_state<APG_LAYOUT_AOS, 4>(action, B, b, a);
  wing_step(s, a, k);
  store_state<APG_LAYOUT_AOS, 12>(next, B, b, s);
}

__global__ __launch_bounds__(256) void wing_learnt_step_bwd_kernel(
    const float *__restrict__ state, const float *__restrict__ action,
    WingGeneralConst k, int B, const float *__restrict__ grad_next,
// ... 9 lines not shown
    load_state<APG_LAYOUT_AOS, 4>(action, B, b, a);
    load_state<APG_LAYOUT_AOS, 12>(grad_next, B, b, lam);
    WingAux x;
    wing_rates(s, a, k, x, sd);
    float ga[4] = {0.f, 0.f, 0.f, 0.f};
    wing_step_adjoint(lam, ga, s, x, sd, k, pg);
    if (grad_state) store_state<APG_LAYOUT_AOS, 12>(grad_state, B, b, lam);
    if (grad_action) store_state<APG_LAYOUT_AOS, 4>(grad_action, B, b, ga);
  }
  const int lane = threadIdx.x & 63;
  const int wave = (blockIdx.x * blockDim.x + threadIdx.x) >> 6;
#pragma unroll
  for (int i = 0; i < kWingParamGrads; ++i) {
    float v = pg.v[i];
#pragma unroll
    for (int m = 32; m >= 1; m >>= 1) v += __shfl_xor(v, m, 64);
    if (lane == 0) wave_partials[(size_t)wave * kWingParamGrads + i] = v;
  }
}

__global__ __launch_bounds__(64) void wing_learnt_reduce_kernel(
    const float *__restrict__ wave_partials, int waves, float *__restrict__ out) {
  const int i = threadIdx.x;
  if (i >= kWingParamGrads) return;
  float acc = 0.f;
  for (int w = 0; w < waves; ++w) acc += wave_partials[(size_t)w * kWingParamGrads + i];
  out[i] = acc;
}

struct WingLearntRolloutArgs {
  const float *state0, *actions, *ref;
  float *loss_partials, *grad_actions, *grad_state0, *states_out;
  const float *pack;
  ApgWingLossWeights w;
  int B, H;
};

__global__ __launch_bounds__(256) void wing_learnt_rollout_pack_kernel(ApgWingLearnt m, float dt,
                                                                       float *__restrict__ pack) {
  if (threadIdx.x == 0) {
    *reinterpret_cast<WingGeneralConst *>(pack) = wing_learnt_table(m.theta, m.inertia, dt);
    for (int i = (int)(sizeof(WingGeneralConst) / sizeof(float)); i < kWingLearntTableFloats; ++i)
      pack[i] = 0.f;
  }
  for (int t = threadIdx.x; t < kWingResFloats; t += blockDim.x)
    pack[kWingLearntTableFloats + t] = wing_residual_packed(t, m.w1, m.b1, m.w2, m.b2);
}

template <int LAYOUT>
__global__ __launch_bounds__(kWave) void wing_learnt_rollout_kernel(WingLearntRolloutArgs A) {
  extern __shared__ float stash[];
  const int lane = threadIdx.x;
  const int b = blockIdx.x * kWave + lane;
  const bool live = b < A.B;
  const int bb = live ? b : A.B - 1;
  const int H = A.H;
  typedef __attribute__((address_space(4))) const float *cfloat_ptr;
  WingGeneralConstK *kp = (WingGeneralConstK *)A.pack;
  cfloat_ptr rows = (cfloat_ptr)(A.pack + kWingLearntTableFloats);
#define APG_LAUNDER(p) asm volatile("" : "+s"(p))
  const float w_pos = A.w.pos, w_act = A.w.action;
  auto ST = [&](int k, int i) -> float & { return stash[(k * 12 + i) * kWave + lane]; };
  float s[12];
  load_state<LAYOUT, 12>(A.state0, A.B, bb, s);
  float loss = 0.f;
  for (int k = 0; k < H; ++k) {
    float a[4], rp[3];
    load_seq<LAYOUT, 4>(A.actions, A.B, H, 4, bb, k, 0, a);
    load_seq<LAYOUT, 3>(A.ref, A.B, H, 3, bb, k, 0, rp);
#pragma unroll
    for (int i = 0; i < 12; ++i) ST(k, i) = s[i];
    APG_LAUNDER(kp);
    APG_LAUNDER(rows);
    wing_learnt_step(s, a, *kp, rows);
    if (A.states_out && live) store_seq<LAYOUT, 12>(A.states_out, A.B, H, 12, b, k, 0, s);
    float lp = 0.f, la = 0.f;
#pragma unroll
    for (int i = 0; i < 3; ++i) {
      const float dp = s[i] - rp[i], d = a[1 + i] - 0.5f;
      lp += dp * dp, la += d * d;
    }
    loss += w_pos * lp + w_act * la;
  }
  write_wave_partial(A.loss_partials, live ? loss : 0.f, (A.B + kWave - 1) / kWave);

  float lam[12];
#pragma unroll
  for (int i = 0; i < 12; ++i) lam[i] = 0.f;
  float nxt[3] = {s[0], s[1], s[2]};
  for (int k = H - 1; k >= 0; --k) {
    float a[4], rp[3], pre[12];
    load_seq<LAYOUT, 4>(A.actions, A.B, H, 4, bb, k, 0, a);
    load_seq<LAYOUT, 3>(A.ref, A.B, H, 3, bb, k, 0, rp);
#pragma unroll
    for (int i = 0; i < 12; ++i) pre[i] = ST(k, i);
#pragma unroll
    for (int i = 0; i < 3; ++i) lam[i] += 2.f * w_pos * (nxt[i] - rp[i]);
    float ga[4] = {0.f, 2.f * w_act * (a[1] - 0.5f), 2.f * w_act * (a[2] - 0.5f),
                   2.f * w_act * (a[3] - 0.5f)};
    APG_LAUNDER(kp);
    APG_LAUNDER(rows);
    wing_learnt_step_adjoint(lam, ga, pre, a, *kp, rows);
    if (live) store_seq<LAYOUT, 4>(A.grad_actions, A.B, H, 4, b, k, 0, ga);
#pragma unroll
    for (int i = 0; i < 3; ++i) nxt[i] = pre[i];
  }
  if (A.grad_state0 && live) store_state<LAYOUT, 12>(A.grad_state0, A.B, b, lam);
#undef APG_LAUNDER
}

static_assert(kWingFitGW1 == APG_WING_FIT_G_W1 && kWingFitGB1 == APG_WING_FIT_G_B1 &&
                  kWingFitGW2 == APG_WING_FIT_G_W2 && kWingFitGB2 == APG_WING_FIT_G_B2 &&
                  kWingFitGrads == APG_WING_FIT_GRADS && APG_WING_FIT_G_I == 41,
              "apg.h publishes these offsets");
constexpr int kFitBlock = 256, kFitWaves = kFitBlock / kWave;
constexpr int kFitSample = 28;
constexpr int kFitWaveLds = kWingFitUnit * kWave;
static_assert(kFitSample <= kWingFitUnit, "the weight planes re-use the sample planes");
constexpr int kFitNorms = kWingLearntPackFloats, kFitRows = kFitNorms + 16;

__global__ __launch_bounds__(256) void wing_learnt_fit_pack_kernel(ApgWingLearnt m, float dt,
                                                                   float *__restrict__ ws) {
  __shared__ float part[4][256];
  if (threadIdx.x == 0) {
    *reinterpret_cast<WingGeneralConst *>(ws) = wing_learnt_table(m.theta, m.inertia, dt);
    for (int i = (int)(sizeof(WingGeneralConst) / sizeof(float)); i < kWingLearntTableFloats; ++i)
      ws[i] = 0.f;
  }
  for (int t = threadIdx.x; t < kWingResFloats; t += blockDim.x)
    ws[kWingLearntTableFloats + t] = wing_residual_packed(t, m.w1, m.b1, m.w2, m.b2);
  const float *tens[4] = {m.w2, m.b2, m.w1, m.b1};
  const int count[4] = {12 * kWingResHidden, 12, kWingResHidden * 16, kWingResHidden};
#pragma unroll
  for (int q = 0; q < 4; ++q) {
    float acc = 0.f;
    for (int t = threadIdx.x; t < count[q]; t += 256) acc = fmaf(tens[q][t], tens[q][t], acc);
    part[q][threadIdx.x] = acc;
  }
  for (int half = 128; half >= 1; half >>= 1) {
    __syncthreads();
    if ((int)threadIdx.x < half)
#pragma unroll
      for (int q = 0; q < 4; ++q) part[q][threadIdx.x] += part[q][threadIdx.x + half];
  }
  if (threadIdx.x < 4) ws[kFitNorms + threadIdx.x] = sqrtf(part[threadIdx.x][0]);
}

struct WingFitArgs {
  const float *state, *action, *target;
  const float *ws;
  float *loss_partials, *rows;
  WingConst eval;
  int B;
};

template <bool EVAL>
__global__ __launch_bounds__(kFitBlock) void wing_learnt_fit_kernel(WingFitArgs A) {
  __shared__ float smp[kFitWaves][kFitWaveLds];
  __shared__ float head[kFitWaves][kWingFitHead];
  typedef __attribute__((address_space(4))) const float *cfloat_ptr;
  WingGeneralConstK *kp = (WingGeneralConstK *)A.ws;
  cfloat_ptr rows = (cfloat_ptr)(A.ws + kWingLearntTableFloats);
  const int lane = threadIdx.x & (kWave - 1), wl = threadIdx.x >> 6;
  const int b = blockIdx.x * kFitBlock + threadIdx.x;
  const bool live = b < A.B;
  const int bb = live ? b : A.B - 1;
  WingParamGrads pg;
#pragma unroll
  for (int i = 0; i < kWingParamGrads; ++i) pg.v[i] = 0.f;
  float s[12], a[4], tgt[12], lam[12];
  load_state<APG_LAYOUT_AOS, 12>(A.state, A.B, bb, s);
  load_state<APG_LAYOUT_AOS, 4>(A.action, A.B, bb, a);
  if constexpr (EVAL) {
#pragma unroll
    for (int i = 0; i < 12; ++i) tgt[i] = s[i];
    const WingConst &ke = A.eval;
    wing_step(tgt, a, ke);
  } else {
    load_state<APG_LAYOUT_AOS, 12>(A.target, A.B, bb, tgt);
  }
  float loss = wing_learnt_fit_sample(s, a, tgt, *kp, rows, lam, pg);
  if (!live) {
    loss = 0.f;
#pragma unroll
    for (int i = 0; i < 12; ++i) lam[i] = 0.f;
#pragma unroll
    for (int i = 0; i < kWingParamGrads; ++i) pg.v[i] = 0.f;
  }
  write_wave_partial(A.loss_partials, loss, (A.B + kWave - 1) / kWave);
#pragma unroll
  for (int i = 0; i < kWingParamGrads; ++i) {
    const float v = wave_sum(pg.v[i]);
    if (lane == 0) head[wl][i] = v;
  }
#pragma unroll
  for (int o = 0; o < 12; ++o) {
    const float v = wave_sum(lam[o]);
    if (lane == 0) head[wl][kWingParamGrads + o] = v;
  }
  if (lane < 2) head[wl][kWingParamGrads + 12 + lane] = 0.f;
  float *mine = smp[wl];
#pragma unroll
  for (int j = 0; j < 12; ++j) mine[j * kWave + lane] = s[j];
#pragma unroll
  for (int j = 0; j < 4; ++j) mine[(12 + j) * kWave + lane] = a[j];
#pragma unroll
  for (int o = 0; o < 12; ++o) mine[(16 + o) * kWave + lane] = lam[o];
  __syncthreads();
  float w[kWingResRow], gw[kWingFitUnit];
  {
    const float4 *src = reinterpret_cast<const float4 *>(A.ws + kWingLearntTableFloats +
                                                         lane * kWingResRow);
#pragma unroll
    for (int q = 0; q < kWingResRow / 4; ++q) {
      const float4 v = src[q];
      w[4 * q] = v.x, w[4 * q + 1] = v.y, w[4 * q + 2] = v.z, w[4 * q + 3] = v.w;
    }
  }
#pragma unroll
  for (int j = 0; j < kWingFitUnit; ++j) gw[j] = 0.f;
#pragma unroll 2
  for (int n = 0; n < kWave; ++n) {
    float zn[16], ln[12];
#pragma unroll
    for (int j = 0; j < 16; ++j) zn[j] = mine[j * kWave + n];
#pragma unroll
    for (int o = 0; o < 12; ++o) ln[o] = mine[(16 + o) * kWave + n];
    wing_residual_unit_grads(w, zn, ln, gw);
  }
  __syncthreads();
#pragma unroll
  for (int j = 0; j < kWingFitUnit; ++j) mine[j * kWave + lane] = gw[j];
  __syncthreads();
  float *row = A.rows + (size_t)blockIdx.x * kWingFitRow;
  for (int c = threadIdx.x; c < kWingFitRow; c += kFitBlock) {
    float acc;
    if (c < kWingFitHead) {
      acc = head[0][c];
#pragma unroll
      for (int v = 1; v < kFitWaves; ++v) acc += head[v][c];
    } else {
      acc = smp[0][c - kWingFitHead];
#pragma unroll
      for (int v = 1; v < kFitWaves; ++v) acc += smp[v][c - kWingFitHead];
    }
    row[c] = acc;
  }
}

constexpr int kFitCols = 32, kFitSplit = 8;
__global__ __launch_bounds__(kFitCols * kFitSplit) void wing_learnt_fit_reduce_kernel(
    const float *__restrict__ ws, int nrows, ApgWingLearnt m, float l2_lambda,
    float *__restrict__ grad, float *__restrict__ loss) {
  __shared__ float part[kFitSplit][kFitCols];
  const int col = threadIdx.x % kFitCols, r = threadIdx.x / kFitCols;
  const int c = blockIdx.x * kFitCols + col;
  const float *rows = ws + kFitRows;
  float acc = 0.f;
#pragma unroll 4
  for (int i = r; i < nrows; i += kFitSplit) acc += rows[(size_t)i * kWingFitRow + c];
  part[r][col] = acc;
  __syncthreads();
  if (r == 0) {
    const float v = ((part[0][col] + part[1][col]) + (part[2][col] + part[3][col])) +
                    ((part[4][col] + part[5][col]) + (part[6][col] + part[7][col]));
    const int dest = wing_fit_dest(c);
    if (dest >= 0) {
      float reg = 0.f;
      if (l2_lambda > 0.f)
        reg = wing_fit_l2_grad(dest, l2_lambda, m.w1, m.b1, m.w2, m.b2, ws + kFitNorms);
      grad[dest] = v + reg;
    }
// ... 201 lines not shown
```

### include/apg.h

```cpp
#ifndef APG_H_
#define APG_H_

#ifdef __cplusplus
extern "C" {
#endif

#define APG_VERSION_MAJOR 0
#define APG_VERSION_MINOR 1

typedef void *apg_stream_t;
typedef void *apg_event_t;

enum { APG_LAYOUT_SOA = 0, APG_LAYOUT_AOS = 1, APG_LAYOUT_PACKED = 2 };

enum {
  APG_OK = 0,
  APG_ERR_ARG = -1,
  APG_ERR_HIP = -2,
  APG_ERR_NO_DEVICE = -3
};

#ifndef APG_ROLLOUT_BLOCK
#define APG_ROLLOUT_BLOCK 64
#endif
// ... 450 lines not shown
  const float *b3;
  const float *w_out;
  const float *b_out;
} ApgCartpolePolicy;

enum { APG_CARTPOLE_BALANCE = 0, APG_CARTPOLE_SWINGUP = 1 };

int apg_cartpole_policy_workspace_floats(void);
int apg_cartpole_mlp_closed_loop(const float *state0, float dt,
                                 const ApgCartpoleParams *params,
                                 const ApgCartpolePolicy *policy, int B, int max_steps,
                                 int mode, float thresh_div, int burn_in, int *steps,
                                 int *upright, double *vel_sum, double *vel_sq,
                                 float *states, float *actions, float *workspace,
                                 apg_stream_t stream);

typedef struct ApgCartpoleLearnt {
  const float *max_force_mag, *masspole, *length, *friction, *total_mass,
      *polemass_length, *w1, *b1, *w2;
} ApgCartpoleLearnt;

int apg_cartpole_learnt_param_count(void);
int apg_cartpole_learnt_workspace_floats(int B);
int apg_cartpole_learnt_step_fwd(const float *state, const float *action, float dt,
                                 const ApgCartpoleLearnt *model, int B, float *next_state,
                                 apg_stream_t stream);
int apg_cartpole_learnt_step_bwd(const float *state, const float *action, float dt,
                                 const ApgCartpoleLearnt *model, int B,
                                 const float *grad_next, float *grad_state,
                                 float *grad_action, float *grad_params, float *workspace,
                                 apg_stream_t stream);

int apg_cartpole_learnt_rollout_fwd_bwd(const float *state0, const float *actions, float dt,
                                        const ApgCartpoleLearnt *model, int B, int H,
                                        int layout, float *loss_partials, float *loss,
                                        float *grad_actions, float *grad_state0,
                                        float *states_out, apg_stream_t stream);

int apg_cartpole_learnt_mlp_closed_loop(const float *state0, float dt,
                                        const ApgCartpoleLearnt *model,
                                        const ApgCartpolePolicy *policy, int B,
                                        int max_steps, int mode, float thresh_div,
                                        int burn_in, int *steps, int *upright,
                                        double *vel_sum, double *vel_sq, float *states,
                                        float *actions, float *workspace,
                                        apg_stream_t stream);

typedef struct ApgCartpoleMpcOptions {
  int iters;
  float beta, alpha;
} ApgCartpoleMpcOptions;

int apg_cartpole_mpc_solve(const float *state0, const float *u0, float dt,
                           const ApgCartpoleParams *model, const ApgCartpoleMpcOptions *opt,
                           int B, int H, float *u, float *cost_out, float *cost_trace,
                           apg_stream_t stream);

int apg_cartpole_mpc_closed_loop(const float *state0, float dt, const ApgCartpoleParams *plant,
                                 const ApgCartpoleLearnt *plant_learnt,
                                 const ApgCartpoleParams *model,
                                 const ApgCartpoleMpcOptions *opt, int B, int H, int max_steps,
                                 int mode, float thresh_div, int burn_in, int *steps,
                                 int *upright, double *vel_sum, double *vel_sq, float *states,
                                 float *actions, float *cost, apg_stream_t stream);

int apg_reduce_loss_partials(const float *partials, int n, float *loss,
                             apg_stream_t stream);
int apg_to_soa(const float *src, const long long *index, int B, int R, int ld,
               float *dst, apg_stream_t stream);
#define APG_SOA_MAX_ITEMS 6
typedef struct ApgSoaItem {
  const float *src;
  const long long *index;
  float *dst;
  int R, ld;
} ApgSoaItem;
int apg_to_soa_multi(const ApgSoaItem *items, int n, int B, apg_stream_t stream);
int apg_loss_partials_count(int B);
int apg_stream_copy(const void *src, void *dst, long long bytes, apg_stream_t stream);
int apg_stream_copy_shape(const void *src, void *dst, long long bytes, int shape,
                          apg_stream_t stream);
int apg_stream_rows_probe(const void *in, long long in_bytes, void *out, long long out_bytes,
                          int shape, apg_stream_t stream);

int apg_version(void);
const char *apg_last_error_string(void);

#ifdef __cplusplus
}
#endif
#endif
```

Before: 77.37 billion env-steps/s.

## Use DPP/permlane wave reductions and move deferred-loss reduction earlier in rollout

Replaces shfl_xor-based wave sums, which go through LDS bpermute, with DPP and permlane16/32 swap intrinsics that keep the reduction in ALU lanes, for both float and double. The deferred reduction of the previous step's loss partials moves from the kernel tail into the forward phase so it overlaps other work. Asm pins are added to keep the scheduler from reordering register state and accumulators. It also makes the wave index compile-time from block size, clamps partial loads branchlessly, and adds a probe entry point for validating the new sums.

```diff
diff --git a/apg_trajectory_tracking_amd/_capi.py b/apg_trajectory_tracking_amd/_capi.py
--- a/apg_trajectory_tracking_amd/_capi.py
+++ b/apg_trajectory_tracking_amd/_capi.py
@@ -363,6 +363,7 @@
     "apg_stream_copy": [_P, _P, ctypes.c_longlong, _P],
     "apg_stream_copy_shape": [_P, _P, ctypes.c_longlong, _I, _P],
     "apg_stream_rows_probe": [_P, ctypes.c_longlong, _P, ctypes.c_longlong, _I, _P],
+    "apg_wave_sum_probe": [_P, _P, _I, _P, _P, _P],
     "apg_version": [],
     "apg_last_error_string": [],
 }
diff --git a/apg_trajectory_tracking_amd/csrc/apg_device.h b/apg_trajectory_tracking_amd/csrc/apg_device.h
--- a/apg_trajectory_tracking_amd/csrc/apg_device.h
+++ b/apg_trajectory_tracking_amd/csrc/apg_device.h
@@ -228,17 +228,95 @@
   return (fx2){sqrt_fast(x.x), sqrt_fast(x.y)};
 }
 
-__device__ __forceinline__ float wave_sum(float v) {
+__device__ __forceinline__ float wave_sum_shfl(float v) {
 #pragma unroll
   for (int off = 32; off > 0; off >>= 1) v += __shfl_xor(v, off, kWave);
   return v;
 }
-
+__device__ __forceinline__ double wave_sum_shfl(double v) {
+#pragma unroll
+  for (int off = 32; off > 0; off >>= 1) v += __shfl_xor(v, off, kWave);
+  return v;
+}
+
+#if defined(__HIP_DEVICE_COMPILE__)
+template <int OFF>
+__device__ __forceinline__ void lane_pair_u32(unsigned x, unsigned &lo, unsigned &hi) {
+  static_assert(OFF == 32 || OFF == 16, "half and row swaps");
+  if constexpr (OFF == 32) {
+    const auto r = __builtin_amdgcn_permlane32_swap(x, x, false, false);
+    lo = r[0], hi = r[1];
+  } else {
+    const auto r = __builtin_amdgcn_permlane16_swap(x, x, false, false);
+    lo = r[0], hi = r[1];
+  }
+}
+template <int OFF>
+__device__ __forceinline__ unsigned lane_xor_u32(unsigned x) {
+  if constexpr (OFF == 8) {
+    return (unsigned)__builtin_amdgcn_update_dpp(0, (int)x, 0x128, 0xf, 0xf, false);
+  } else if constexpr (OFF == 4) {
+    int t = __builtin_amdgcn_update_dpp(0, (int)x, 0x104, 0xf, 0x5, false);
+    t = __builtin_amdgcn_update_dpp(t, (int)x, 0x114, 0xf, 0xa, false);
+    return (unsigned)t;
+  } else if constexpr (OFF == 2) {
+    return (unsigned)__builtin_amdgcn_update_dpp(0, (int)x, 0x4e, 0xf, 0xf, false);
+  } else {
+    static_assert(OFF == 1, "DPP partners: 8, 4, 2, 1");
+    return (unsigned)__builtin_amdgcn_update_dpp(0, (int)x, 0xb1, 0xf, 0xf, false);
+  }
+}
+template <int OFF>
+__device__ __forceinline__ float add_lane_xor(float v) {
+  const unsigned x = __builtin_bit_cast(unsigned, v);
+  if constexpr (OFF >= 16) {
+    unsigned lo, hi;
+    lane_pair_u32<OFF>(x, lo, hi);
+    return __builtin_bit_cast(float, lo) + __builtin_bit_cast(float, hi);
+  } else {
+    return v + __builtin_bit_cast(float, lane_xor_u32<OFF>(x));
+  }
+}
+template <int OFF>
+__device__ __forceinline__ double add_lane_xor(double v) {
+  const unsigned long long u = __builtin_bit_cast(unsigned long long, v);
+  const unsigned w0 = (unsigned)u, w1 = (unsigned)(u >> 32);
+  auto f64 = [](unsigned a, unsigned b) {
+    return __builtin_bit_cast(double, ((unsigned long long)b << 32) | a);
+  };
+  if constexpr (OFF >= 16) {
+    unsigned lo0, hi0, lo1, hi1;
+    lane_pair_u32<OFF>(w0, lo0, hi0);
+    lane_pair_u32<OFF>(w1, lo1, hi1);
+    return f64(lo0, lo1) + f64(hi0, hi1);
+  } else {
+    return v + f64(lane_xor_u32<OFF>(w0), lane_xor_u32<OFF>(w1));
+  }
+}
+template <typename T>
+__device__ __forceinline__ T wave_sum_alu(T v) {
+  v = add_lane_xor<32>(v);
+  v = add_lane_xor<16>(v);
+  v = add_lane_xor<8>(v);
+  v = add_lane_xor<4>(v);
+  v = add_lane_xor<2>(v);
+  v = add_lane_xor<1>(v);
+  return v;
+}
+__device__ __forceinline__ float wave_sum(float v) { return wave_sum_alu(v); }
+__device__ __forceinline__ double wave_sum(double v) { return wave_sum_alu(v); }
+#else
+__device__ __forceinline__ float wave_sum(float v) { return wave_sum_shfl(v); }
+__device__ __forceinline__ double wave_sum(double v) { return wave_sum_shfl(v); }
+#endif
+
+template <int BLOCK>
 __device__ __forceinline__ void write_wave_partial(float *partials, float lane_loss,
                                                    int count = 0x7fffffff) {
+  static_assert(BLOCK > 0 && BLOCK % kWave == 0, "whole waves");
   float s = wave_sum(lane_loss);
   if ((threadIdx.x & (kWave - 1)) == 0) {
-    int wave = (blockIdx.x * blockDim.x + threadIdx.x) / kWave;
+    const int wave = blockIdx.x * (BLOCK / kWave) + threadIdx.x / kWave;
     if (wave < count) partials[wave] = s;
   }
 }
@@ -252,31 +330,47 @@
                                                  PrevPartials &pp) {
   const int lane = threadIdx.x & (kWave - 1);
   pp.acc = 0.0;
+  const int last = d.prev_count - 1;
   for (int base = 16 * kWave; base < d.prev_count; base += 16 * kWave) {
     float t[16];
 #pragma unroll
     for (int j = 0; j < 16; ++j) {
       const int i = base + j * kWave + lane;
-      t[j] = i < d.prev_count ? d.prev_partials[i] : 0.f;
-    }
-#pragma unroll
-    for (int j = 0; j < 16; ++j) pp.acc += (double)t[j];
-  }
-#pragma unroll
-  for (int j = 0; j < 16; ++j) {
-    const int i = j * kWave + lane;
-    pp.v[j] = i < d.prev_count ? d.prev_partials[i] : 0.f;
+      t[j] = d.prev_partials[i < last ? i : last];
+    }
+#pragma unroll
+    for (int j = 0; j < 16; ++j) {
+      const int i = base + j * kWave + lane;
+      pp.acc += (double)(i <= last ? t[j] : 0.f);
+    }
+  }
+#pragma unroll
+  for (int j = 0; j < 16; ++j) pp.v[j] = 0.f;
+  if (d.prev_count > 0) {
+#pragma unroll
+    for (int j = 0; j < 16; ++j) {
+      const int i = j * kWave + lane;
+      pp.v[j] = d.prev_partials[i < last ? i : last];
+    }
   }
 }
 
 __device__ __forceinline__ void reduce_prev_tail(const ApgDeferredLoss &d,
                                                  const PrevPartials &pp) {
+  const int lane = threadIdx.x & (kWave - 1);
+  float v[16];
+#pragma unroll
+  for (int j = 0; j < 16; ++j) v[j] = pp.v[j];
+  asm volatile(""
+               : "+v"(v[0]), "+v"(v[1]), "+v"(v[2]), "+v"(v[3]), "+v"(v[4]), "+v"(v[5]),
+                 "+v"(v[6]), "+v"(v[7]), "+v"(v[8]), "+v"(v[9]), "+v"(v[10]), "+v"(v[11]),
+                 "+v"(v[12]), "+v"(v[13]), "+v"(v[14]), "+v"(v[15]));
   double acc = pp.acc;
 #pragma unroll
-  for (int j = 0; j < 16; ++j) acc += (double)pp.v[j];
-#pragma unroll
-  for (int off = 32; off > 0; off >>= 1) acc += __shfl_xor(acc, off, kWave);
-  if ((threadIdx.x & (kWave - 1)) == 0) d.prev_loss[0] = (float)acc;
+  for (int j = 0; j < 16; ++j)
+    acc += (double)(j * kWave + lane < d.prev_count ? v[j] : 0.f);
+  acc = wave_sum(acc);
+  if (lane == 0) d.prev_loss[0] = (float)acc;
 }
 
 __device__ __forceinline__ void reduce_prev_partials(const ApgDeferredLoss &d) {
diff --git a/apg_trajectory_tracking_amd/csrc/cartpole.hip b/apg_trajectory_tracking_amd/csrc/cartpole.hip
--- a/apg_trajectory_tracking_amd/csrc/cartpole.hip
+++ b/apg_trajectory_tracking_amd/csrc/cartpole.hip
@@ -76,7 +76,7 @@
     }
     loss += 0.01f * a[0] * a[0];
   }
-  write_wave_partial(A.loss_partials, live ? loss : 0.f, (A.B + kWave - 1) / kWave);
+  write_wave_partial<APG_ROLLOUT_BLOCK>(A.loss_partials, live ? loss : 0.f, (A.B + kWave - 1) / kWave);
 
   float lam[4] = {0.f, 0.f, 0.f, 0.f}, g0[4] = {0.f, 0.f, 0.f, 0.f};
   float nxt[4] = {s[0], s[1], s[2], s[3]};
diff --git a/apg_trajectory_tracking_amd/csrc/cartpole_learnt.hip b/apg_trajectory_tracking_amd/csrc/cartpole_learnt.hip
--- a/apg_trajectory_tracking_amd/csrc/cartpole_learnt.hip
+++ b/apg_trajectory_tracking_amd/csrc/cartpole_learnt.hip
@@ -156,7 +156,7 @@
     }
     loss += 0.01f * a[0] * a[0];
   }
-  write_wave_partial(A.loss_partials, live ? loss : 0.f, (A.B + kWave - 1) / kWave);
+  write_wave_partial<APG_ROLLOUT_BLOCK>(A.loss_partials, live ? loss : 0.f, (A.B + kWave - 1) / kWave);
 
   float lam[4] = {0.f, 0.f, 0.f, 0.f}, g0[4] = {0.f, 0.f, 0.f, 0.f};
   float nxt[4] = {s[0], s[1], s[2], s[3]};
diff --git a/apg_trajectory_tracking_amd/csrc/common.hip b/apg_trajectory_tracking_amd/csrc/common.hip
--- a/apg_trajectory_tracking_amd/csrc/common.hip
+++ b/apg_trajectory_tracking_amd/csrc/common.hip
@@ -182,8 +182,31 @@
   }
 }
 
+static __global__ __launch_bounds__(256) void wave_sum_probe_kernel(
+    const float *__restrict__ in32, const double *__restrict__ in64, int n,
+    float *__restrict__ out32, double *__restrict__ out64) {
+  const int i = blockIdx.x * 256 + threadIdx.x;
+  if (i >= n) return;
+  const float f = in32[i];
+  const double d = in64[i];
+  out32[i] = apg::wave_sum_shfl(f);
+  out32[n + i] = apg::wave_sum(f);
+  out64[i] = apg::wave_sum_shfl(d);
+  out64[n + i] = apg::wave_sum(d);
+}
 
 extern "C" {
+
+int apg_wave_sum_probe(const float *in32, const double *in64, int n, float *out32,
+                       double *out64, apg_stream_t stream) {
+  if (!in32 || !in64 || !out32 || !out64 || n <= 0 || n % apg::kWave) {
+    apg::set_error("apg_wave_sum_probe: non-NULL pointers and n a positive multiple of 64");
+    return APG_ERR_ARG;
+  }
+  hipLaunchKernelGGL(wave_sum_probe_kernel, dim3((n + 255) / 256), dim3(256), 0,
+                     (hipStream_t)stream, in32, in64, n, out32, out64);
+  return apg::check_launch("wave_sum_probe");
+}
 
 int apg_stream_rows_probe(const void *in, long long in_bytes, void *out, long long out_bytes,
                           int shape, apg_stream_t stream) {
diff --git a/apg_trajectory_tracking_amd/csrc/lstm.hip b/apg_trajectory_tracking_amd/csrc/lstm.hip
--- a/apg_trajectory_tracking_amd/csrc/lstm.hip
+++ b/apg_trajectory_tracking_amd/csrc/lstm.hip
@@ -826,7 +826,7 @@
   if (live && A.grad_c0)
 #pragma unroll
     for (int r = 0; r < 4; ++r) A.grad_c0[(size_t)(r + 4 * hi) * B + b] = dc[r];
-  write_wave_partial(A.loss_partials, st_lo ? loss : 0.f);
+  write_wave_partial<kThreads>(A.loss_partials, st_lo ? loss : 0.f);
   if (A.cot_amax) {
     float mg = run_g, mz = run_z;
 #pragma unroll
diff --git a/apg_trajectory_tracking_amd/csrc/mlp_concurrent_fwd.h b/apg_trajectory_tracking_amd/csrc/mlp_concurrent_fwd.h
--- a/apg_trajectory_tracking_amd/csrc/mlp_concurrent_fwd.h
+++ b/apg_trajectory_tracking_amd/csrc/mlp_concurrent_fwd.h
@@ -365,7 +365,7 @@
     const float v = hi ? act[(row + 4) >> 2][(row + 4) & 3] : act[row >> 2][row & 3];
     Pdz.st(vr, row * pN, v);
   }
-  write_wave_partial(A.loss_partials, st_lo ? loss : 0.f);
+  write_wave_partial<kThreads>(A.loss_partials, st_lo ? loss : 0.f);
 }
 
 }
diff --git a/apg_trajectory_tracking_amd/csrc/mlp_planes.hip b/apg_trajectory_tracking_amd/csrc/mlp_planes.hip
--- a/apg_trajectory_tracking_amd/csrc/mlp_planes.hip
+++ b/apg_trajectory_tracking_amd/csrc/mlp_planes.hip
@@ -216,7 +216,7 @@
   if (st_lo && A.grad_state0)
 #pragma unroll
     for (int i = 0; i < 12; ++i) A.grad_state0[(size_t)i * B + b] = lam[i];
-  write_wave_partial(A.loss_partials, st_lo ? loss : 0.f);
+  write_wave_partial<kThreads>(A.loss_partials, st_lo ? loss : 0.f);
 }
 
 __global__ __launch_bounds__(kThreads) void mlp_concurrent_bwd_kernel(ConcArgs A) {
diff --git a/apg_trajectory_tracking_amd/csrc/mlp_rollout.hip b/apg_trajectory_tracking_amd/csrc/mlp_rollout.hip
--- a/apg_trajectory_tracking_amd/csrc/mlp_rollout.hip
+++ b/apg_trajectory_tracking_amd/csrc/mlp_rollout.hip
@@ -930,7 +930,7 @@
   if (st_lo && A.grad_state0)
 #pragma unroll
     for (int i = 0; i < 12; ++i) A.grad_state0[(size_t)i * B + b] = lam[i];
-  write_wave_partial(A.loss_partials, st_lo ? loss : 0.f);
+  write_wave_partial<kThreads>(A.loss_partials, st_lo ? loss : 0.f);
 }
 
 }
diff --git a/apg_trajectory_tracking_amd/csrc/quad.hip b/apg_trajectory_tracking_amd/csrc/quad.hip
--- a/apg_trajectory_tracking_amd/csrc/quad.hip
+++ b/apg_trajectory_tracking_amd/csrc/quad.hip
@@ -60,6 +60,15 @@
 #define APG_STAMP_FLUSH()
 #endif
 
+#define APG_PIN_SUMS(a, b, c, d, e) \
+  asm volatile("" : "+v"(a), "+v"(b), "+v"(c), "+v"(d), "+v"(e))
+#define APG_PIN_SUM(a) asm volatile("" : "+v"(a))
+#define APG_PIN_STATE(s)                                                        \
+  asm volatile(""                                                              \
+               : "+v"(s[0]), "+v"(s[1]), "+v"(s[2]), "+v"(s[3]), "+v"(s[4]),   \
+                 "+v"(s[5]), "+v"(s[6]), "+v"(s[7]), "+v"(s[8]), "+v"(s[9]),   \
+                 "+v"(s[10]), "+v"(s[11]))
+
 template <int LAYOUT>
 __global__ __launch_bounds__(256) void quad_step_fwd_kernel(
     const float *__restrict__ state, const float *__restrict__ action,
@@ -192,6 +201,8 @@
       __builtin_amdgcn_sched_barrier(0);
     }
   }
+  if (reducer) reduce_prev_tail(A.prev, pp);
+  __builtin_amdgcn_sched_barrier(0);
 
   Trig st_trig[HT];
   float st_w[HT + 1][3];
@@ -267,6 +278,7 @@
       sum_r = fmaf(d, d, sum_r);
       ga[i] = wr2 * d;
     }
+    APG_PIN_SUMS(sum_p, sum_v, sum_w, sum_r, sum_t);
     quad_step_adjoint(lam, ga, a0, st_w[k], c, st_trig[k]);
     if (live) {
       if constexpr (BUF) {
@@ -289,8 +301,8 @@
   APG_STAMP_AT(3);
   const float loss = A.w.pos * sum_p + A.w.vel * sum_v + A.w.av * sum_w +
                      A.w.rates * sum_r + A.w.thrust * sum_t;
-  write_wave_partial(A.loss_partials, live ? loss : 0.f, (A.B + kWave - 1) / kWave);
-  if (reducer) reduce_prev_tail(A.prev, pp);
+  write_wave_partial<APG_ROLLOUT_BLOCK>(A.loss_partials, live ? loss : 0.f,
+                                        (A.B + kWave - 1) / kWave);
   APG_STAMP_FLUSH();
 }
 
@@ -403,6 +415,7 @@
   PrevPartials pp;
   if (reducer) reduce_prev_head(R.prev, pp);
   __builtin_amdgcn_sched_barrier(0);
+  constexpr int kReduceAt = kActPre < HT ? kActPre : HT;
 
   float s[12];
   Trig st_trig[HT];
@@ -425,6 +438,11 @@
       }
       __builtin_amdgcn_sched_barrier(0);
     }
+    if (k == kReduceAt && k > 0) {
+      APG_PIN_STATE(s);
+      if (reducer) reduce_prev_tail(R.prev, pp);
+      __builtin_amdgcn_sched_barrier(0);
+    }
     if (k == 0) {
 #pragma unroll
       for (int g = 0; g < 3; ++g) {
@@ -450,6 +468,11 @@
             r_so, st16, (k * 3 + g) * p16, 2);
     }
     if (k == 0) APG_STAMP_AT(1);
+  }
+  if constexpr (kReduceAt == HT) {
+    APG_PIN_STATE(s);
+    if (reducer) reduce_prev_tail(R.prev, pp);
+    __builtin_amdgcn_sched_barrier(0);
   }
 #pragma unroll
   for (int i = 0; i < 3; ++i) st_w[HT][i] = s[9 + i];
@@ -497,6 +520,7 @@
       sum_r = fmaf(d, d, sum_r);
       ga[i] = wr2 * d;
     }
+    APG_PIN_SUMS(sum_p, sum_v, sum_w, sum_r, sum_t);
     quad_step_adjoint(lam, ga, a0, st_w[k], c, st_trig[k]);
     if constexpr (kStoreAtEnd) {
       constexpr int kFlush = kStoreFlushAt;
@@ -534,8 +558,7 @@
   APG_STAMP_AT(3);
   const float loss = R.w.pos * sum_p + R.w.vel * sum_v + R.w.av * sum_w +
                      R.w.rates * sum_r + R.w.thrust * sum_t;
-  write_wave_partial(R.loss_partials, live ? loss : 0.f, (B + kWave - 1) / kWave);
-  if (reducer) reduce_prev_tail(R.prev, pp);
+  write_wave_partial<kBlock>(R.loss_partials, live ? loss : 0.f, (B + kWave - 1) / kWave);
   APG_STAMP_FLUSH();
 }
 
@@ -582,6 +605,7 @@
     __builtin_amdgcn_raw_ptr_buffer_load_lds(
         r_ref, (lds_ptr)(l_ref + i * 256), 16, lane * 16,
         blockIdx.x * (64 * RC * HT * 4) + i * 1024, 0, 0);
+  if (reducer) reduce_prev_tail(A.prev, pp);
   asm volatile("s_waitcnt vmcnt(%0)" ::"n"(kRefChunks) : "memory");
 
   float s[12];
@@ -644,6 +668,7 @@
     }
     loss += A.w.pos * lp + A.w.vel * lv + A.w.av * lw + A.w.rates * lr +
             A.w.thrust * da0 * da0;
+    APG_PIN_SUM(loss);
     quad_step_adjoint(lam, ga, a0, st_w[k], c, st_trig[k]);
     *reinterpret_cast<float4 *>(&l_act[lane * 4 * HT + 4 * k]) =
         make_float4(ga[0], ga[1], ga[2], ga[3]);
@@ -659,8 +684,8 @@
   }
   if (A.grad_state0 && live)
     store_state<APG_LAYOUT_AOS, 12>(A.grad_state0, A.B, b, lam);
-  write_wave_partial(A.loss_partials, live ? loss : 0.f, (A.B + kWave - 1) / kWave);
-  if (reducer) reduce_prev_tail(A.prev, pp);
+  write_wave_partial<APG_ROLLOUT_BLOCK>(A.loss_partials, live ? loss : 0.f,
+                                        (A.B + kWave - 1) / kWave);
 }
 
 template <int LAYOUT, bool STATES_OUT>
@@ -708,7 +733,8 @@
     loss += A.w.pos * lp + A.w.vel * lv + A.w.av * lw + A.w.rates * lr +
             A.w.thrust * da0 * da0;
   }
-  write_wave_partial(A.loss_partials, live ? loss : 0.f, (A.B + kWave - 1) / kWave);
+  write_wave_partial<APG_ROLLOUT_BLOCK>(A.loss_partials, live ? loss : 0.f,
+                                        (A.B + kWave - 1) / kWave);
 
   float lam[12], wn[3] = {s[9], s[10], s[11]};
 #pragma unroll
@@ -911,7 +937,8 @@
   }
   const float loss = A.w.pos * sum_p + A.w.vel * sum_v + A.w.av * sum_w +
                      A.w.rates * sum_r + A.w.thrust * sum_t;
-  write_wave_partial(A.loss_partials, live ? loss : 0.f, (A.B + kWave - 1) / kWave);
+  write_wave_partial<APG_ROLLOUT_BLOCK>(A.loss_partials, live ? loss : 0.f,
+                                        (A.B + kWave - 1) / kWave);
 
   float lam[12], nxt[12];
 #pragma unroll
@@ -990,7 +1017,7 @@
     if (live && grad_actions)
       store_seq<LAYOUT, 4>(grad_actions, B, H, 4, b, k, 0, ga);
   }
-  write_wave_partial(partials, live ? loss : 0.f, (B + kWave - 1) / kWave);
+  write_wave_partial<APG_ROLLOUT_BLOCK>(partials, live ? loss : 0.f, (B + kWave - 1) / kWave);
 }
 
 template <int LAYOUT>
diff --git a/apg_trajectory_tracking_amd/csrc/wing.hip b/apg_trajectory_tracking_amd/csrc/wing.hip
--- a/apg_trajectory_tracking_amd/csrc/wing.hip
+++ b/apg_trajectory_tracking_amd/csrc/wing.hip
@@ -155,7 +155,7 @@
     }
     loss += w_pos * lp + w_act * la;
   }
-  write_wave_partial(A.loss_partials, live ? loss : 0.f, (A.B + kWave - 1) / kWave);
+  write_wave_partial<APG_ROLLOUT_BLOCK>(A.loss_partials, live ? loss : 0.f, (A.B + kWave - 1) / kWave);
 
   float lam[12];
 #pragma unroll
diff --git a/apg_trajectory_tracking_amd/csrc/wing_learnt.hip b/apg_trajectory_tracking_amd/csrc/wing_learnt.hip
--- a/apg_trajectory_tracking_amd/csrc/wing_learnt.hip
+++ b/apg_trajectory_tracking_amd/csrc/wing_learnt.hip
@@ -115,7 +115,7 @@
     }
     loss += w_pos * lp + w_act * la;
   }
-  write_wave_partial(A.loss_partials, live ? loss : 0.f, (A.B + kWave - 1) / kWave);
+  write_wave_partial<kWave>(A.loss_partials, live ? loss : 0.f, (A.B + kWave - 1) / kWave);
 
   float lam[12];
 #pragma unroll
@@ -220,7 +220,7 @@
 #pragma unroll
     for (int i = 0; i < kWingParamGrads; ++i) pg.v[i] = 0.f;
   }
-  write_wave_partial(A.loss_partials, loss, (A.B + kWave - 1) / kWave);
+  write_wave_partial<kFitBlock>(A.loss_partials, loss, (A.B + kWave - 1) / kWave);
 #pragma unroll
   for (int i = 0; i < kWingParamGrads; ++i) {
     const float v = wave_sum(pg.v[i]);
diff --git a/include/apg.h b/include/apg.h
--- a/include/apg.h
+++ b/include/apg.h
@@ -556,6 +556,8 @@
                           apg_stream_t stream);
 int apg_stream_rows_probe(const void *in, long long in_bytes, void *out, long long out_bytes,
                           int shape, apg_stream_t stream);
+int apg_wave_sum_probe(const float *in32, const double *in64, int n, float *out32,
+                       double *out64, apg_stream_t stream);
 
 int apg_version(void);
 const char *apg_last_error_string(void);
```

After: 77.55 billion env-steps/s, median of 3. No clear change (+0.2%).
